# vanilladucky/sde_sampler_lrds

Hardware: NVIDIA B200
Metric: particle_steps_per_sec (higher is better)
Workload: dtype f32

## Files before the change

### sde_sampler_lrds_b200/csrc/lrds_rollout_mix.cuh

```cuda
#pragma once
#include "lrds_rollout_tc.cuh"

namespace lrds {

constexpr int MIX_MAX_WARPS = 16;
constexpr int MIX_TAIL_BYTES = 32;
constexpr float MIX_LOGIT_KAPPA = 9.5367431640625e-07f;
constexpr float MIX_LOGIT_KAPPA_C = 2.384185791015625e-07f;
constexpr float MIX_LOGIT_TAU = 2e-5f;

template <bool EUBO_, int TGT_, int REF_, bool EM_, bool DIS_ = false>
struct MixCfg {
  static constexpr bool kEubo = EUBO_, kEm = EM_, kDis = DIS_;
  static constexpr int kTgt = TGT_, kRef = REF_;
};
using MixBench = MixCfg<false, 1, 2, false>;

__host__ __device__ inline int mix_tc_config(const lrds_spec& s) {
  if (s.precision != LRDS_PRECISION_F16X3 || s.mlp.d_pad > 128 || gmm_full_on_path(s)) return -1;
  const bool tmix = s.ctrl_kind == LRDS_CTRL_SCORE && s.target.kind == LRDS_DISTR_GMM && s.target.gmm.M > 1 &&
                    s.target.gmm.M <= MIX_MAX_M && s.target.gmm.mix_tc != nullptr;
  const bool tdis = s.ctrl_kind >= LRDS_CTRL_CANCEL_DRIFT && s.target.kind == LRDS_DISTR_GMM && s.target.gmm.M > 1 &&
                    s.target.gmm.M <= MIX_MAX_M && s.target.gmm.mix_tc != nullptr;
  const bool tphi = s.ctrl_kind == LRDS_CTRL_SCORE && s.target.kind == LRDS_DISTR_PHI4;
  const bool tnone = s.ctrl_kind == LRDS_CTRL_CLIPPED &&
                     (s.target.kind != LRDS_DISTR_GMM || s.target.gmm.M <= MIX_MAX_M) && s.target.kind != LRDS_DISTR_LOGREG;
  const bool rnone = !s.has_ref_ctrl;
  const bool rmix = s.has_ref_ctrl && s.ref_t.M > 1 && s.ref_t.M <= MIX_MAX_M && s.ref_t.mix_tc != nullptr;
  const bool rgauss = s.has_ref_ctrl && s.ref_t.M == 1;
  const bool axpy = s.update_form == LRDS_UPDATE_AXPY && (s.ito_form == LRDS_ITO_SCALED || (rnone && s.ito_form != LRDS_ITO_EM));
  const bool em = s.update_form == LRDS_UPDATE_EM && (s.ito_form == LRDS_ITO_EM || (rnone && s.ito_form == LRDS_ITO_NONE));
  if (s.ref_0.M > MIX_MAX_M) return -1;
  if (s.target.kind == LRDS_DISTR_GMM && s.target.gmm.M > 1 && s.target.gmm.mix_tc == nullptr) return -1;
  if (s.kind == LRDS_ROLLOUT_EUBO_LINEAR) return (tmix && rmix && axpy) ? 1 : -1;
  if (s.kind != LRDS_ROLLOUT_LINEAR) return -1;
  if (tmix && rmix && axpy) return 0;
  if (tmix && rgauss && axpy) return 2;
  if (tmix && rgauss && em) return 3;
  if (tphi && rmix && axpy) return 4;
  if (tnone && rmix && axpy) return 5;
  if (tmix && rmix && em) return 6;
  if (tmix && rnone && em) return 7;
  if (tmix && rnone && axpy) return 8;
  if (tphi && rgauss && axpy) return 9;
  if (tdis && rnone && em) return 10;
  return -1;
}
__host__ __device__ inline bool mix_tc_applicable(const lrds_spec& s) { return mix_tc_config(s) >= 0; }

__device__ __forceinline__ float gmm_logp_any(const GmmView& g, int d, int dp, const Col4& x) {
  if (g.M == 1) {
    const int nq = (d + 3) >> 2;
    float q = 0.f;
    for (int c = 0; c < nq; ++c) quad4(q, x.ld4(c), g.mu.ld4(c), g.ivar.ld4(c));
    return g.glogc.ld1(0) - 0.5f * q;
  }
  float r[MIX_MAX_M];
  return gmm_pass1_pair(g, d, dp, x, r);
}

#ifdef LRDS_MIX_TIMING
static __device__ unsigned long long g_mix_timing[2 * 16 * 16];
struct MixTm {
  unsigned long long* w = nullptr;
  long long t;
  __device__ __forceinline__ void start() { t = clock64(); }
  __device__ __forceinline__ void mark(int i) {
    const long long n = clock64();
    if (w != nullptr && (threadIdx.x & 31) == 0) w[i] += (unsigned long long)(n - t);
    t = n;
  }
  __device__ __forceinline__ void count(int i, bool hit) {
    if (w != nullptr && (threadIdx.x & 31) == 0 && hit) w[i] += 1ull;
  }
};
#else
struct MixTm {
  __device__ __forceinline__ void start() {}
  __device__ __forceinline__ void mark(int) {}
  __device__ __forceinline__ void count(int, bool) {}
};
#endif

template <int PREC>
struct MixTc : TcMlp<PREC> {
  using Base = TcMlp<PREC>;
  static constexpr uint32_t kRCol = 0, kDCol = 32;
  uint32_t lbo, part_bytes;
  uint32_t lg_part;
  MixTm tm;

  __device__ __forceinline__ void logit(int which, uint32_t img, int col = -1) const {
    const uint32_t dcol = this->tm_tile + (col < 0 ? this->d_col() : (uint32_t)col) + (uint32_t)which * MIX_MAX_M;
    mma_passes<true, true>(dcol, this->tm_tile + this->a_col(0), this->tm_tile + this->a_col(1), 8u, img, lg_part,
                           2u * MIX_MAX_M * 16u, MIX_MAX_M * 16u, 128u, this->L.Kin / 16, ptx::make_idesc_f16(128, MIX_MAX_M));
  }
  template <bool TGT, bool REF>
  __device__ __forceinline__ void chunk(int c, uint32_t tgt_img, uint32_t ref_img, uint32_t col = kDCol, uint32_t rcol = kRCol) const {
    const uint32_t idesc = ptx::make_idesc_f16(128, 16);
#pragma unroll
    for (int which = TGT ? 0 : 1; which < (REF ? 2 : 1); ++which) {
      const uint32_t img = (which ? ref_img : tgt_img) + (uint32_t)c * 256u;
      const uint32_t dcol = this->tm_tile + col + which * 16;
      const uint32_t a_hi = this->tm_tile + rcol + which * 16, a_lo = a_hi + 8;
      const uint64_t b_hi = ptx::make_smem_desc(img, lbo, 128u), b_lo = ptx::make_smem_desc(img + part_bytes, lbo, 128u);
      ptx::mma_bf16_ts(dcol, a_lo, b_hi, idesc, 0);
      ptx::mma_bf16_ts(dcol, a_hi, b_lo, idesc, 1);
      ptx::mma_bf16_ts(dcol, a_hi, b_hi, idesc, 1);
    }
  }

  static __device__ __forceinline__ void pack_r(const float (&r)[MIX_MAX_M], uint32_t (&p)[16]) {
#pragma unroll
    for (int i = 0; i < 8; ++i) {
      u64 hi, lo;
      f2::split(f2::pack(r[2 * i], r[2 * i + 1]), hi, lo);
      float h0, h1, l0, l1;
      f2::unpack(hi, h0, h1);
      f2::unpack(lo, l0, l1);
      p[i] = ptx::pack_f16x2(h0, h1);
      p[8 + i] = ptx::pack_f16x2(l0, l1);
    }
  }
  __device__ __forceinline__ void store_r(int which, const uint32_t (&p)[16], uint32_t rcol = kRCol) {
    ptx::tmem_st16(this->tm_lane + rcol + which * 16, p);
  }
  __device__ __forceinline__ void load_chunk(uint32_t (&m)[32]) {
    ptx::tmem_ld32(this->tm_lane + kDCol, m);
    ptx::tmem_wait_ld();
  }

  static __device__ __forceinline__ bool softmax_logits(const uint32_t* acc, const PPtr<true>& tail, float xnorm, uint32_t (&p)[16]) {
    float r[MIX_MAX_M];
    const float4 t2 = tail.ld4(MIX_MAX_M / 4);
#pragma unroll
    for (int q = 0; q < MIX_MAX_M / 4; ++q) {
      const float4 c = tail.ld4(q);
      r[4 * q + 0] = fmaf(__uint_as_float(acc[4 * q + 0]), t2.x, c.x);
      r[4 * q + 1] = fmaf(__uint_as_float(acc[4 * q + 1]), t2.x, c.y);
      r[4 * q + 2] = fmaf(__uint_as_float(acc[4 * q + 2]), t2.x, c.z);
      r[4 * q + 3] = fmaf(__uint_as_float(acc[4 * q + 3]), t2.x, c.w);
    }
    float mx = r[0];
#pragma unroll
    for (int i = 1; i < MIX_MAX_M; ++i) mx = fmaxf(mx, r[i]);
    float s = 0.f;
#pragma unroll
    for (int mb = 0; mb < MIX_MAX_M / 4; ++mb) {
#pragma unroll
      for (int i = 0; i < 4; ++i) r[4 * mb + i] = __expf(r[4 * mb + i] - mx);
      s += (r[4 * mb] + r[4 * mb + 1]) + (r[4 * mb + 2] + r[4 * mb + 3]);
    }
    const float inv = 1.0f / s;
#pragma unroll
    for (int i = 0; i < MIX_MAX_M; ++i) r[i] *= inv;
    pack_r(r, p);
    const float eps = fmaf(MIX_LOGIT_KAPPA * xnorm, t2.y, MIX_LOGIT_KAPPA_C * t2.z);
    const float amb = fminf(1.0f, 4.0f * (s - 1.0f) * inv);
    return eps * amb <= MIX_LOGIT_TAU && xnorm < 3.0e4f;
  }

  template <bool BIAS_SH, class S0, class S1>
  __device__ __forceinline__ void hidden_ws(const float* __restrict__ bias1, S0&& slot0, S1&& slot1) {
    const TcLayout& L = this->L;
    this->issue(L.off_in, L.Kin, C);
    tm.mark(1);
    slot0();
    tm.mark(2);
    const float* bh = reinterpret_cast<const float*>(this->img + L.off_bhid);
    const int nh = L.nh;
    for (int l = 0; l <= nh; ++l) {
      if (l == 1) {
        slot1();
        tm.mark(5);
      }
      this->wait();
      tm.mark(l == 0 ? 3 : l == 1 ? 6 : 8);
      if (l == 0) this->template epilogue_f16<!BIAS_SH>(bias1, 0);
      else this->template epilogue_f16<false>(bh + (l - 1) * C, l);
      if (l < nh) this->issue(L.off_hid + (uint32_t)(l * C * C * L.es), C, C);
      else this->issue(L.off_out, C, L.Nout);
      tm.mark(l == 0 ? 4 : 7);
    }
    if (nh == 0) slot1();
    this->wait();
    tm.mark(8);
  }
};

template <bool RMIX>
__device__ __forceinline__ void mix_load_step(const lrds_spec& s, const StageLayout& SL, uint8_t* stage, int k) {
  uint64_t* sbar = reinterpret_cast<uint64_t*>(stage) + (k & 1);
  uint8_t* dst = stage + SL.off_buf + (k & 1) * SL.buf_bytes;
  const bool tgt = k == 0 && SL.tgt_bytes;
  ptx::mbar_expect_tx(sbar, SL.buf_bytes + (tgt ? SL.tgt_bytes : 0u));
  if (tgt) {
    stage_gmm(stage + SL.off_tgt, gmm_at(s.target.gmm, 0), SL.tgt_logc_bytes, SL.tgt_param_bytes, sbar);
    ptx::bulk_g2s(stage + SL.off_tgt + SL.tgt_logc_bytes + SL.tgt_param_bytes, static_cast<const uint8_t*>(s.target.gmm.mix_tc),
                  SL.tgt_mix_bytes, sbar);
  }
  stage_step(dst, s, SL, k, sbar);
  if constexpr (RMIX)
    ptx::bulk_g2s(dst + SL.row_bytes + SL.ref_logc_bytes + SL.ref_param_bytes,
                  static_cast<const uint8_t*>(s.ref_t.mix_tc) + (int64_t)k * s.ref_t.step_stride_mix_tc, SL.ref_mix_bytes, sbar);
}

template <int PREC, class CFG>
__device__ __forceinline__ void rollout_body_mix(const RolloutArgs& a, float* smem, uint8_t* stage, uint32_t* step_cnt, const int nwarps,
                                                 MixTc<PREC>& mlp) {
  constexpr bool EUBO = CFG::kEubo, TMIX = CFG::kTgt == 1, TPHI = CFG::kTgt == 2, RMIX = CFG::kRef == 2, RGAUSS = CFG::kRef == 1, EM = CFG::kEm, DIS = CFG::kDis;
  const lrds_spec& s = a.s;
  const int NT = nwarps * 32;
  const int tid = threadIdx.x;
  const int b_raw = blockIdx.x * NT + tid;
  const bool live = b_raw < s.B;
  const int b = live ? b_raw : s.B - 1;
  const int d = s.d, dp = s.mlp.d_pad, K = s.K;
  const ColLayout L = col_layout(s, true);
  const Particle P = make_particle(smem, L, NT, tid);

  for (int j = 0; j < dp; ++j) P.x(j) = (j < d) ? __ldg(a.x0 + (int64_t)b * d + j) : 0.f;
  if (!EUBO && a.traj_out != nullptr && live)
    for (int j = 0; j < d; ++j) a.traj_out[(int64_t)b * d + j] = P.x(j);

  CtrlConst cc = ctrl_const(s);
  const GmmView tv0 = gmm_at(s.target.gmm, 0);
  const StageLayout SL = stage_layout(s, 2, true);
  uint64_t* sbar = reinterpret_cast<uint64_t*>(stage);
  const uint32_t mix_off_t = SL.tgt_logc_bytes + SL.tgt_param_bytes;
  const uint32_t mix_off_r = SL.row_bytes + SL.ref_logc_bytes + SL.ref_param_bytes;
  const int Mt = TMIX ? s.target.gmm.M : s.ref_t.M;
  const uint32_t contr_bytes = gmm_mix_contr_bytes(Mt, dp), lg_part = gmm_mix_logit_part_bytes(Mt, dp);
  const uint32_t lg_tail_off = contr_bytes + 2u * lg_part;
  const GmmViewT<true> tv = staged_view(stage + SL.off_tgt, tv0, SL.tgt_logc_bytes, SL.tgt_param_bytes);
  const uint32_t tgt_img = ptx::smem_u32(stage + SL.off_tgt + mix_off_t);
  mlp.lbo = (uint32_t)(2 * dp) * 16u;
  mlp.part_bytes = (contr_bytes - 16u) / 2u;
  mlp.lg_part = lg_part;
  auto target_logp = [&]() -> float {
    if (s.target.kind == LRDS_DISTR_GMM) {
      if (s.target.gmm.M == 1) return gmm_logp_any(tv0, d, dp, P.x);
      float rt[MIX_MAX_M];
      return gmm_pass1_pair(tv, d, dp, P.x, rt);
    }
    if (s.target.kind == LRDS_DISTR_PHI4) return phi4_logp(s.target.phi4, d, P.x);
    return 0.f;
  };
  const float coef = s.target.phi4.a * (float)d, beta = s.target.phi4.beta;
  const u64 p0 = f2::pk(-beta * s.target.phi4.b / coef), p1 = f2::pk(beta / coef), p3 = f2::pk(-beta / coef),
            pn = f2::pk(beta * coef), m2 = f2::pk(-2.0f);
  const int nchunk = dp / JC;
  const int nq = (d + 3) >> 2;
  float rnd = 0.f;
  __syncwarp();
  if constexpr (EUBO) {
    ptx::mbar_wait(sbar, 0);
    const float lref = gmm_logp_any(gmm_at(s.ref_0, 0), d, dp, P.x);
    rnd = lref - clipf(target_logp(), s.clip_target);
  }

  mlp.tm.start();
  for (int k = 0; k < K; ++k) {
    ptx::mbar_wait(sbar + (k & 1), (uint32_t)(k >> 1) & 1u);
    mlp.tm.mark(0);
    const uint8_t* buf = stage + SL.off_buf + (k & 1) * SL.buf_bytes;
    const float* row = reinterpret_cast<const float*>(buf);
    const PPtr<true> rowp{ptx::smem_u32(buf)};
    const GmmViewT<true> rv = staged_view(buf + SL.row_bytes, gmm_at(s.ref_t, k), SL.ref_logc_bytes, SL.ref_param_bytes);
    const uint32_t ref_img = ptx::smem_u32(buf + mix_off_r);
    const float A = rowp.ld1(LRDS_STEP_A), Bc = rowp.ld1(LRDS_STEP_B), Cc = rowp.ld1(LRDS_STEP_C);
    const float wcost = rowp.ld1(LRDS_STEP_W_COST), wito = rowp.ld1(LRDS_STEP_W_ITO);
    const float gamma = rowp.ld1(LRDS_STEP_GAMMA);
    const float ust = TMIX ? *reinterpret_cast<const float*>(stage + SL.off_tgt + mix_off_t + contr_bytes - 16u) : 1.0f;
    const float usr = RMIX ? *reinterpret_cast<const float*>(buf + mix_off_r + contr_bytes - 16u) : 1.0f;
    const GmmView rg = gmm_at(s.ref_t, k);

    if constexpr (EUBO) {
      const u64 mean2 = f2::pk(rowp.ld1(LRDS_STEP_EU_A)), std2 = f2::pk(rowp.ld1(LRDS_STEP_EU_B));
      for (int c = 0; c < nchunk; ++c) {
        float z[JC];
        noise_chunk(a, k, b, c * JC, z);
        const ulonglong2 xa = P.x.ldu(2 * c), xb = P.x.ldu(2 * c + 1);
        P.x.stu(2 * c, ulonglong2{f2::fma(std2, f2::pack(z[0], z[1]), f2::mul(xa.x, mean2)),
                                  f2::fma(std2, f2::pack(z[2], z[3]), f2::mul(xa.y, mean2))});
        P.x.stu(2 * c + 1, ulonglong2{f2::fma(std2, f2::pack(z[4], z[5]), f2::mul(xb.x, mean2)),
                                      f2::fma(std2, f2::pack(z[6], z[7]), f2::mul(xb.y, mean2))});
      }
    }
    mlp.store_x(P.x);
    uint32_t rt_p[16], rr_p[16];
    bool need_t = TMIX, need_r = RMIX;
    bool ok_t = false, ok_r = false;
    if constexpr (TMIX || RMIX) {
      const PPtr<true> tail_t{tgt_img + lg_tail_off}, tail_r{ref_img + lg_tail_off};
      const bool lg_t = TMIX && tail_t.ld1(MIX_MAX_M + 3) != 0.f, lg_r = RMIX && tail_r.ld1(MIX_MAX_M + 3) != 0.f;
      if (lg_t || lg_r) {
        mlp.arrive_issue([&]() {
          if (lg_t) mlp.logit(0, tgt_img + contr_bytes);
          if (lg_r) mlp.logit(1, ref_img + contr_bytes);
        });
        u64 n2 = 0;
        for (int c = 0; c < nq; ++c) {
          const ulonglong2 xv = P.x.ldu(c);
          n2 = f2::fma(xv.x, xv.x, n2);
          n2 = f2::fma(xv.y, xv.y, n2);
        }
        const float xnorm = sqrtf(f2::hsum1(n2));
        mlp.wait();
        uint32_t lg[32];
        ptx::tmem_ld32(mlp.tm_lane + mlp.d_col(), lg);
        ptx::tmem_wait_ld();
        if (lg_t) {
          ok_t = mlp.softmax_logits(lg, tail_t, xnorm, rt_p);
          need_t = __any_sync(0xffffffffu, !ok_t);
        }
        if (lg_r) {
          ok_r = mlp.softmax_logits(lg + MIX_MAX_M, tail_r, xnorm, rr_p);
          need_r = __any_sync(0xffffffffu, !ok_r);
        }
      }
    }
    mlp.tm.count(14, need_t);
    mlp.tm.count(15, need_r);
    mlp.template hidden_ws<true>(
        row + LRDS_STEP_BIAS1,
        [&]() {
          if constexpr (TMIX) {
            if (need_t) {
              float r[MIX_MAX_M];
              uint32_t p[16];
              gmm_pass1_pair(tv, d, dp, P.x, r);
              mlp.pack_r(r, p);
#pragma unroll
              for (int i = 0; i < 16; ++i) rt_p[i] = ok_t ? rt_p[i] : p[i];
            }
          }
        },
        [&]() {
          if constexpr (RMIX) {
            if (need_r) {
              float r[MIX_MAX_M];
              uint32_t p[16];
              gmm_pass1_pair(rv, d, dp, P.x, r);
              mlp.pack_r(r, p);
#pragma unroll
              for (int i = 0; i < 16; ++i) rr_p[i] = ok_r ? rr_p[i] : p[i];
            }
          }
        });
    if constexpr (TMIX) mlp.store_r(0, rt_p);
    if constexpr (RMIX) mlp.store_r(1, rr_p);
    mlp.arrive_issue([&]() { mlp.template chunk<TMIX, RMIX>(0, tgt_img, ref_img); });
    mlp.tm.mark(9);
    const float dt = EM ? rowp.ld1(LRDS_STEP_DT) : 0.f, sqdt = EM ? rowp.ld1(LRDS_STEP_SQRT_DT) : 0.f;
    const u64 A2 = f2::pk(EM ? 1.0f - A * dt : A), B2 = f2::pk(EM ? Bc * dt : Bc), C2 = f2::pk(EM ? Bc * sqdt : Cc);
    const u64 usr2 = f2::pk(usr), R2 = f2::pk((EM ? Cc * dt : Bc) * usr);
    const bool lerp = DIS && s.ctrl_kind == LRDS_CTRL_LERP;
    const float gsc = DIS ? rowp.ld1(LRDS_STEP_GSCALE) : 1.0f, wl = DIS ? rowp.ld1(LRDS_STEP_LERP) : 0.f;
    const u64 cx2 = f2::pk(DIS ? rowp.ld1(LRDS_STEP_CX) : 0.f), ust2 = f2::pk(ust);
    const u64 wl2 = f2::pk(wl < 0.5f ? wl : -(1.0f - wl));
    const GmmView pg = gmm_at(s.ref_0, 0);
    const u64 gs2 = f2::pk(((cc.scale_score * gamma) * gsc) * (lerp ? 1.0f : ust));
    const float bts = lerp ? cc.bound_score : cc.bound_score / ust;
    const float wz = EM ? (s.ito_form == LRDS_ITO_NONE ? 0.f : sqdt)
                     : (RMIX || RGAUSS || s.ito_form == LRDS_ITO_SCALED) ? wito
                     : s.ito_form == LRDS_ITO_DDS ? rowp.ld1(LRDS_STEP_SIGU) * wito
                                                  : 0.f;
    u64 su2 = 0, sito = 0;
    float xm = 0.f;
    for (int c = 0; c < nchunk; ++c) {
      const int j0 = c * JC;
      uint32_t m[32];
      mlp.wait();
      mlp.tm.mark(10);
      mlp.load_chunk(m);
      if (c + 1 < nchunk) mlp.arrive_issue([&]() { mlp.template chunk<TMIX, RMIX>(c + 1, tgt_img, ref_img); });
      mlp.tm.mark(11);
      const ulonglong2 xa = P.x.ldu(2 * c), xb = P.x.ldu(2 * c + 1);
      const u64 X[4] = {xa.x, xa.y, xb.x, xb.y};
      u64 U[4], XN[4];
      float z[JC];
      mlp.out_chunk2(j0, U);
      noise_chunk(a, k, b, j0, z);
      float xs[JC + 2];
      if constexpr (TPHI) {
        xs[0] = xm;
#pragma unroll
        for (int q = 0; q < 4; ++q) f2::unpack(X[q], xs[1 + 2 * q], xs[2 + 2 * q]);
        xs[JC + 1] = (j0 + JC < dp) ? P.x(j0 + JC) : 0.f;
        xm = xs[JC];
      }
      u64 GM[4], GI[4];
      if constexpr (RGAUSS) {
        const ulonglong2 g0 = rg.mu.ld2(2 * c), g1 = rg.mu.ld2(2 * c + 1), i0 = rg.ivar.ld2(2 * c), i1 = rg.ivar.ld2(2 * c + 1);
        GM[0] = g0.x; GM[1] = g0.y; GM[2] = g1.x; GM[3] = g1.y;
        GI[0] = i0.x; GI[1] = i0.y; GI[2] = i1.x; GI[3] = i1.y;
      }
      if constexpr (DIS) {
        if (lerp) {
          const ulonglong2 g0 = pg.mu.ld2(2 * c), g1 = pg.mu.ld2(2 * c + 1), i0 = pg.ivar.ld2(2 * c), i1 = pg.ivar.ld2(2 * c + 1);
          GM[0] = g0.x; GM[1] = g0.y; GM[2] = g1.x; GM[3] = g1.y;
          GI[0] = i0.x; GI[1] = i0.y; GI[2] = i1.x; GI[3] = i1.y;
        }
      }
#pragma unroll
      for (int q = 0; q < 4; ++q) {
        const u64 ta = f2::pack(__uint_as_float(m[2 * q]), __uint_as_float(m[2 * q + 1]));
        const u64 tb = f2::pack(__uint_as_float(m[8 + 2 * q]), __uint_as_float(m[9 + 2 * q]));
        const u64 ra = f2::pack(__uint_as_float(m[16 + 2 * q]), __uint_as_float(m[17 + 2 * q]));
        const u64 rb = f2::pack(__uint_as_float(m[24 + 2 * q]), __uint_as_float(m[25 + 2 * q]));
        float t0 = 0.f, t1 = 0.f, u0, u1;
        if constexpr (TMIX) f2::unpack(f2::fma(X[q], ta, tb), t0, t1);
        if constexpr (DIS) {
          if (lerp) {
            const u64 tt = f2::mul(f2::pack(t0, t1), ust2);
            const u64 pr = f2::mul(f2::fma(X[q], f2::pk(-1.0f), GM[q]), GI[q]);
            const u64 df = f2::fma(pr, f2::pk(-1.0f), tt);
            f2::unpack(f2::fma(df, wl2, wl < 0.5f ? pr : tt), t0, t1);
          }
        }
        if constexpr (TPHI) {
          const u64 nb = f2::pack(xs[2 * q] + xs[2 * q + 2], xs[2 * q + 1] + xs[2 * q + 3]);
          const u64 t = f2::fma(X[q], f2::fma(f2::mul(X[q], X[q]), p3, p1), f2::fma(pn, f2::fma(X[q], m2, nb), p0));
          f2::unpack(t, t0, t1);
          if (j0 + JC > d) {
            if (j0 + 2 * q >= d) t0 = 0.f;
            if (j0 + 2 * q + 1 >= d) t1 = 0.f;
          }
        }
        f2::unpack(U[q], u0, u1);
        const u64 uc = f2::pack(clipb(u0, cc.bound_model), clipb(u1, cc.bound_model));
        u64 v = uc;
        if constexpr (DIS) v = f2::fma(X[q], cx2, v);
        if constexpr (TMIX || TPHI) v = f2::fma(f2::pack(clipb(t0, bts), clipb(t1, bts)), gs2, v);
        const u64 rraw = RMIX ? f2::fma(X[q], ra, rb) : RGAUSS ? f2::mul(f2::fma(X[q], f2::pk(-1.0f), GM[q]), GI[q]) : 0ull;
        const u64 z2 = f2::pack(z[2 * q], z[2 * q + 1]);
        if constexpr (EUBO) {
          su2 = f2::fma(v, f2::fma(v, f2::pk(0.5f), f2::mul(rraw, usr2)), su2);
          sito = f2::fma(v, z2, sito);
          continue;
        }
        su2 = f2::fma(v, v, su2);
        sito = f2::fma(v, z2, sito);
        if constexpr (!RMIX && !RGAUSS) {
          XN[q] = f2::fma(C2, z2, f2::fma(A2, X[q], f2::mul(B2, v)));
        } else if constexpr (EM) {
          XN[q] = f2::fma(C2, z2, f2::fma(A2, X[q], f2::fma(R2, rraw, f2::mul(B2, v))));
        } else {
          const u64 rv2 = f2::fma(rraw, usr2, v);
          XN[q] = f2::fma(C2, z2, f2::fma(A2, X[q], f2::mul(B2, rv2)));
        }
      }
      if constexpr (EUBO) {
        mlp.tm.mark(12);
        continue;
      }
      P.x.stu(2 * c, ulonglong2{XN[0], XN[1]});
      P.x.stu(2 * c + 1, ulonglong2{XN[2], XN[3]});
      if (a.traj_out != nullptr && live) {
        float xn[JC];
#pragma unroll
        for (int q = 0; q < 4; ++q) f2::unpack(XN[q], xn[2 * q], xn[2 * q + 1]);
        store_traj(a, k + 1, b, j0, xn);
      }
      mlp.tm.mark(12);
    }
    if constexpr (EUBO) {
      rnd -= f2::hsum1(su2) * wcost;
      rnd -= f2::hsum1(sito) * wito;
    } else {
      rnd += wcost * f2::hsum1(su2);
      rnd += wz * f2::hsum1(sito);
    }
    __syncwarp();
    if ((tid & 31) == 0) {
      const uint32_t old = ptx::atom_add_acq_rel(step_cnt + (k & 1), 1u);
      if (old == (uint32_t)((k >> 1) * nwarps + nwarps - 1) && k + 2 < K) mix_load_step<RMIX>(s, SL, stage, k + 2);
    }
    mlp.tm.mark(13);
  }
  __syncwarp();
  if constexpr (!EUBO) {
    const float lref = s.init_cost ? a.rnd_out[b] : gmm_logp_any(gmm_at(s.ref_0, 0), d, dp, P.x);
    rnd += lref - clipf(target_logp(), s.clip_target);
  }

  float xsum = 0.f;
  if (live) {
    a.rnd_out[b] = rnd;
    if (a.x_out != nullptr)
      for (int j = 0; j < d; ++j) {
        const float v = P.x(j);
        xsum += v;
        a.x_out[(int64_t)b * d + j] = v;
      }
  }
  report_status(s, live, mlp.saturated(), !isfinite(rnd + xsum));
}

template <int PREC, class CFG>
__device__ __forceinline__ void mix_aux_issuer(const RolloutArgs& a, uint8_t* stage, MixTc<PREC>& mlp) {
  constexpr bool TMIX = CFG::kTgt == 1, RMIX = CFG::kRef == 2;
  const lrds_spec& s = a.s;
  const int dp = s.mlp.d_pad, K = s.K, nchunk = dp / JC, nh = mlp.L.nh;
  const StageLayout SL = stage_layout(s, 2, true);
  uint64_t* sbar = reinterpret_cast<uint64_t*>(stage);
  const uint32_t mix_off_t = SL.tgt_logc_bytes + SL.tgt_param_bytes;
  const uint32_t mix_off_r = SL.row_bytes + SL.ref_logc_bytes + SL.ref_param_bytes;
  const int Mt = TMIX ? s.target.gmm.M : s.ref_t.M;
  const uint32_t contr_bytes = gmm_mix_contr_bytes(Mt, dp), lg_part = gmm_mix_logit_part_bytes(Mt, dp);
  const uint32_t lg_tail_off = contr_bytes + 2u * lg_part;
  const uint32_t tgt_img = ptx::smem_u32(stage + SL.off_tgt + mix_off_t);
  mlp.lbo = (uint32_t)(2 * dp) * 16u;
  mlp.part_bytes = (contr_bytes - 16u) / 2u;
  mlp.lg_part = lg_part;
  const TcLayout& L = mlp.L;
  for (int k = 0; k < K; ++k) {
    ptx::mbar_wait(sbar + (k & 1), (uint32_t)(k >> 1) & 1u);
    const uint8_t* buf = stage + SL.off_buf + (k & 1) * SL.buf_bytes;
    const uint32_t ref_img = ptx::smem_u32(buf + mix_off_r);
    if constexpr (TMIX || RMIX) {
      const PPtr<true> tail_t{tgt_img + lg_tail_off}, tail_r{ref_img + lg_tail_off};
      const bool lg_t = TMIX && tail_t.ld1(MIX_MAX_M + 3) != 0.f, lg_r = RMIX && tail_r.ld1(MIX_MAX_M + 3) != 0.f;
      if (lg_t || lg_r)
        mlp.issue_when_ready([&]() {
          if (lg_t) mlp.logit(0, tgt_img + contr_bytes);
          if (lg_r) mlp.logit(1, ref_img + contr_bytes);
        });
    }
    mlp.issue_when_ready([&]() { mlp.gemm(L.off_in, L.Kin, C); });
    for (int l = 0; l < nh; ++l) mlp.issue_when_ready([&]() { mlp.gemm(L.off_hid + (uint32_t)(l * C * C * L.es), C, C); });
    mlp.issue_when_ready([&]() { mlp.gemm(L.off_out, C, L.Nout); });
    for (int c = 0; c < nchunk; ++c) mlp.issue_when_ready([&]() { mlp.template chunk<TMIX, RMIX>(c, tgt_img, ref_img); });
  }
}

template <int PREC, class CFG>
__global__ void __launch_bounds__(MIX_MAX_WARPS * 32, 1)
rollout_mix_kernel(const RolloutArgs a, const uint8_t* __restrict__ image, const uint32_t tmem_cols, const int nwarps) {
  extern __shared__ __align__(128) uint8_t smem_raw[];
  constexpr bool RMIX = CFG::kRef == 2;
  const lrds_spec& s = a.s;
  const TcLayout TL = tc_layout(s.d, s.mlp.num_hidden, PREC);
  const int tid = threadIdx.x;
  const int warp = __shfl_sync(0xffffffffu, tid >> 5, 0);
  const bool has_aux = (int)(blockDim.x >> 5) > nwarps;
  uint64_t* bars = reinterpret_cast<uint64_t*>(smem_raw + TL.bytes);
  uint32_t* cnts = reinterpret_cast<uint32_t*>(smem_raw + TL.bytes + TC_TAIL_BYTES);
  uint8_t* stage = smem_raw + TL.bytes + TC_TAIL_BYTES + MIX_TAIL_BYTES;
  const StageLayout SL = stage_layout(s, 2, true);
  float* cols = reinterpret_cast<float*>(stage + ((SL.total + 15u) & ~15u));
  auto steps01 = [&]() {
    for (int k = 0; k < 2 && k < s.K; ++k) mix_load_step<RMIX>(s, SL, stage, k);
  };
  const uint32_t tmem = __shfl_sync(
      0xffffffffu, tc_cta_begin(smem_raw, TL, image, tmem_cols, warp, 5, reinterpret_cast<uint64_t*>(stage), 2, cnts, 6, 0u, steps01), 0);
  const bool aux = warp == nwarps;
  const int tile = aux ? (nwarps - 1) >> 2 : warp >> 2;
  const int tile_warps = min(4, nwarps - 4 * tile);
  uint32_t issue_mask = ((warp & 3) == tile_warps - 1 ? 1u : 0u) | ((warp & 3) == max(tile_warps - 2, 0) ? 2u : 0u);
  if (has_aux && tile_warps < 4) issue_mask = 0u;
  MixTc<PREC> mlp;
  mlp.init(TL, smem_raw, tmem + (uint32_t)(tile * TL.tile_cols), warp, bars + 1 + tile, cnts + tile, (uint32_t)tile_warps, issue_mask,
           s.mlp.d_pad);
#ifdef LRDS_MIX_TIMING
  unsigned long long* tmw = reinterpret_cast<unsigned long long*>(cols + (size_t)col_layout(s, true).total * 32 * nwarps) + warp * 16;
  if ((tid & 31) < 16) tmw[tid & 31] = 0;
  __syncwarp();
  mlp.tm.w = tmw;
#endif
  if (aux) mix_aux_issuer<PREC, CFG>(a, stage, mlp);
  else rollout_body_mix<PREC, CFG>(a, cols, stage, cnts + 4, nwarps, mlp);
#ifdef LRDS_MIX_TIMING
  __syncwarp();
  if ((blockIdx.x == 0 || blockIdx.x == gridDim.x / 2) && (tid & 31) < 16)
    g_mix_timing[((blockIdx.x ? 1 : 0) * 16 + warp) * 16 + (tid & 31)] = tmw[tid & 31];
#endif
  tc_cta_end(warp, tmem, tmem_cols);
}

inline bool plan_rollout_mix(const lrds_spec& s, int smem_cap, int sms, TcPlan* out) {
  if (!mix_tc_applicable(s)) return false;
  const TcLayout TL = tc_layout(s.d, s.mlp.num_hidden, s.precision);
  if (TL.tile_cols > 512 || TL.parts * TL.a_cols < 64) return false;
  const ColLayout CL = col_layout(s, true);
  size_t fixed = (size_t)TL.bytes + TC_TAIL_BYTES + MIX_TAIL_BYTES + ((stage_layout(s, 2, true).total + 15u) & ~15u);
#ifdef LRDS_MIX_TIMING
  fixed += 16 * 16 * 8;
#endif
  const size_t per_warp = (size_t)CL.total * 32 * sizeof(float);
  if (fixed + per_warp > (size_t)smem_cap) return false;
  int wmax = (int)(((size_t)smem_cap - fixed) / per_warp);
  wmax = wmax < MIX_MAX_WARPS ? wmax : MIX_MAX_WARPS;
  wmax = wmax < 4 * (512 / TL.tile_cols) ? wmax : 4 * (512 / TL.tile_cols);
  const int need = (s.B + 31) / 32;
  const int w = plan_warps(need, sms, wmax);
  out->warps = w;
  out->grid = (need + w - 1) / w;
  out->staged = 2;
  out->tmem_cols = plan_tmem_cols((w + 3) / 4 * TL.tile_cols);
  out->smem = fixed + per_warp * w;
  return true;
}

template <class CFG>
int launch_mix_cfg(const RolloutArgs& a, const TcPlan& p, cudaStream_t st) {
  const int aux = (p.warps % 4 != 0 && p.warps < MIX_MAX_WARPS) ? 1 : 0;
  return launch_tc(rollout_mix_kernel<LRDS_PRECISION_F16X3, CFG>, "mixture tensor-core rollout", a, p, (p.warps + aux) * 32, st,
                   p.tmem_cols, p.warps);
}

}
```

### sde_sampler_lrds_b200/csrc/lrds_rollout_simt.cuh

```cuda
#pragma once
#include "lrds_device.cuh"
#include "lrds_tc_ptx.cuh"

namespace lrds {

struct RolloutArgs {
  lrds_spec s;
  const float* x0;
  const float* noise;
  uint64_t seed;
  uint64_t particle_offset;
  float* x_out;
  float* rnd_out;
  float* traj_out;
};

__device__ __forceinline__ void report_status(const lrds_spec& s, bool live, bool saturated, bool nonfinite) {
  if (s.status != nullptr && live) {
    if (saturated) atomicAdd(s.status, 1u);
    if (nonfinite) atomicAdd(s.status + 1, 1u);
  }
}

struct ColLayout {
  int x, act, rt, rr, rh, g, us, tsd, db, total;
};

__host__ __device__ inline bool ref_t_full(const lrds_spec& s) { return s.has_ref_ctrl && s.ref_t.layout == LRDS_GMM_FULL; }
__host__ __device__ inline bool gmm_full_on_path(const lrds_spec& s) {
  return ref_t_full(s) || s.ref_0.layout == LRDS_GMM_FULL || (s.target.kind == LRDS_DISTR_GMM && s.target.gmm.layout == LRDS_GMM_FULL);
}

__host__ __device__ inline ColLayout col_layout(const lrds_spec& s, bool mix_tc = false) {
  ColLayout L{};
  int off = 0;
  const int dp = s.mlp.d_pad;
  L.x = off; off += dp;
  L.act = off;
  if (s.precision == LRDS_PRECISION_FP32_SIMT) off += C;
  L.rt = off;
  const bool tfull = s.target.kind == LRDS_DISTR_GMM && s.target.gmm.layout == LRDS_GMM_FULL;
  if (!mix_tc && !tfull && s.target.kind == LRDS_DISTR_GMM && s.target.gmm.M > 1) off += (s.target.gmm.M + 3) / 4 * 4;
  L.rr = off;
  L.rh = off;
  if (ref_t_full(s) || tfull) {
    L.rh = off + dp;
    off += 2 * dp;
    if (s.ref_0.layout != LRDS_GMM_FULL && s.ref_0.M > 1 && s.ref_0.M > 2 * dp) off += (s.ref_0.M + 3) / 4 * 4 - 2 * dp;
  } else if (!mix_tc) {
    int m = 0;
    if (s.has_ref_ctrl && s.ref_t.M > 1) m = s.ref_t.M;
    if (s.ref_0.layout != LRDS_GMM_FULL && s.ref_0.M > 1 && s.ref_0.M > m) m = s.ref_0.M;
    off += (m + 3) / 4 * 4;
  }
  L.g = off;
  if (s.target.kind == LRDS_DISTR_LOGREG) off += s.target.logreg.n_pad;
  L.us = off; L.tsd = off; L.db = off;
  if (s.kind == LRDS_ROLLOUT_CMCD || s.kind == LRDS_ROLLOUT_EUBO_CMCD) {
    L.us = off; off += dp;
    L.tsd = off; off += dp;
    L.db = off; off += dp;
  } else if (s.kind == LRDS_ROLLOUT_EUBO_LINEAR) {
    L.db = off; off += dp;
  }
  L.total = off;
  return L;
}

struct Particle {
  Col4 x, rt, rr, rh;
  Col g, us, tsd, db;
};

__device__ __forceinline__ Particle make_particle(float* smem, const ColLayout& L, int NT, int tid) {
  Particle P;
  P.x = Col4{smem + L.x * NT + 4 * tid, 4 * NT};
  P.rt = Col4{smem + L.rt * NT + 4 * tid, 4 * NT};
  P.rr = Col4{smem + L.rr * NT + 4 * tid, 4 * NT};
  P.rh = Col4{smem + L.rh * NT + 4 * tid, 4 * NT};
  P.g = Col{smem + L.g * NT + tid, NT};
  P.us = Col{smem + L.us * NT + tid, NT};
  P.tsd = Col{smem + L.tsd * NT + tid, NT};
  P.db = Col{smem + L.db * NT + tid, NT};
  return P;
}

struct StageLayout {
  uint32_t tgt_logc_bytes, tgt_param_bytes, tgt_bytes;
  uint32_t ref_logc_bytes, ref_param_bytes, row_bytes;
  uint32_t tgt_mix_bytes, ref_mix_bytes;
  uint32_t buf_bytes, off_tgt, off_buf, total;
};
__host__ __device__ inline uint32_t gmm_mix_contr_bytes(int M, int d_pad) {
  return 2u * (uint32_t)((M + 15) / 16 * 2) * (uint32_t)(2 * d_pad) * 16u + 16u;
}
__host__ __device__ inline uint32_t gmm_mix_logit_part_bytes(int M, int d_pad) {
  return (uint32_t)((M + 15) / 16 * 16) * (uint32_t)((d_pad + 15) / 16 * 16) * 2u;
}
__host__ __device__ inline uint32_t gmm_mix_tc_bytes(int M, int d_pad) {
  return gmm_mix_contr_bytes(M, d_pad) + 2u * gmm_mix_logit_part_bytes(M, d_pad) + (uint32_t)((M + 15) / 16 * 16) * 4u + 16u;
}

__host__ __device__ inline StageLayout stage_layout(const lrds_spec& s, int level, bool mix_tc = false) {
  StageLayout L{};
  const uint32_t dp = (uint32_t)s.mlp.d_pad;
  if (level >= 2 && s.target.kind == LRDS_DISTR_GMM && s.target.gmm.M > 1) {
    L.tgt_logc_bytes = (uint32_t)((s.target.gmm.M + 3) / 4 * 4) * 4u;
    L.tgt_param_bytes = (uint32_t)((s.target.gmm.M + 3) / 4) * dp * 32u;
    if (mix_tc) L.tgt_mix_bytes = gmm_mix_tc_bytes(s.target.gmm.M, s.mlp.d_pad);
    L.tgt_bytes = L.tgt_logc_bytes + L.tgt_param_bytes + L.tgt_mix_bytes;
  }
  if (s.has_ref_ctrl && s.ref_t.M > 1 && !ref_t_full(s)) {
    L.ref_logc_bytes = (uint32_t)((s.ref_t.M + 3) / 4 * 4) * 4u;
    L.ref_param_bytes = (uint32_t)((s.ref_t.M + 3) / 4) * dp * 32u;
    if (mix_tc) L.ref_mix_bytes = gmm_mix_tc_bytes(s.ref_t.M, s.mlp.d_pad);
  }
  L.row_bytes = LRDS_STEP_STRIDE * 4u;
  L.buf_bytes = L.row_bytes + L.ref_logc_bytes + L.ref_param_bytes + L.ref_mix_bytes;
  L.off_tgt = 16;
  L.off_buf = L.off_tgt + L.tgt_bytes;
  L.total = L.off_buf + 2u * L.buf_bytes;
  return L;
}

__device__ __forceinline__ void stage_gmm(uint8_t* dst, const GmmView& g, uint32_t logc_bytes, uint32_t param_bytes,
                                          uint64_t* bar) {
  ptx::bulk_g2s(dst, g.logc.p, logc_bytes, bar);
  ptx::bulk_g2s(dst + logc_bytes, g.sn.p, param_bytes, bar);
}
__device__ __forceinline__ void stage_step(uint8_t* dst, const lrds_spec& s, const StageLayout& L, int k, uint64_t* bar) {
  ptx::bulk_g2s(dst, s.steps + (int64_t)k * LRDS_STEP_STRIDE, L.row_bytes, bar);
  if (L.ref_param_bytes) stage_gmm(dst + L.row_bytes, gmm_at(s.ref_t, k), L.ref_logc_bytes, L.ref_param_bytes, bar);
}
__device__ __forceinline__ GmmViewT<true> staged_view(const uint8_t* src, const GmmView& g, uint32_t logc_bytes,
                                                     uint32_t param_bytes) {
  GmmViewT<true> v;
  const uint32_t a = ptx::smem_u32(src);
  v.M = g.M;
  v.logc = PPtr<true>{a};
  v.sn = PPtr<true>{a + logc_bytes};
  v.glogc = g.glogc;
  v.mu = g.mu;
  v.ivar = g.ivar;
  return v;
}

template <int UPDATE = -1, int ITO = -1, int TARGET = -1, int SCORE = -1, int REF = -1, int MIX = 0>
struct LinearTraits {
  static constexpr bool kMix = MIX != 0;
  static constexpr int kUpdate = UPDATE;
  static constexpr int kIto = ITO;
  static constexpr int kTarget = TARGET;
  static constexpr int kScore = SCORE;
  static constexpr int kRef = REF;
};
using RuntimeTraits = LinearTraits<>;
__host__ __device__ inline int ref_class(const lrds_spec& s) {
  return !s.has_ref_ctrl ? 0 : (ref_t_full(s) ? 3 : (s.ref_t.M > 1 ? 2 : 1));
}
template <class TR>
__host__ __device__ inline bool traits_match(const lrds_spec& s) {
  return (TR::kUpdate < 0 || TR::kUpdate == s.update_form) && (TR::kIto < 0 || TR::kIto == s.ito_form) &&
         (TR::kTarget < 0 || TR::kTarget == s.target.kind) &&
         (TR::kScore < 0 || (s.ctrl_kind <= LRDS_CTRL_SCORE && TR::kScore == (s.ctrl_kind == LRDS_CTRL_SCORE))) &&
         (TR::kRef < 0 || TR::kRef == ref_class(s)) && (TR::kRef < 0 || !gmm_full_on_path(s)) &&
         (!TR::kMix || ((s.target.kind != LRDS_DISTR_GMM || s.target.gmm.M > 1) && (!s.has_ref_ctrl || s.ref_t.M > 1)));
}

struct SimtMlp {
  static constexpr bool kPipe = true;
  const lrds_mlp& w;
  Col act;
  template <bool BIAS_SH>
  __device__ __forceinline__ void hidden(const float* __restrict__ bias1, const Col4& x) {
    mlp_hidden<BIAS_SH>(w, bias1, x, act);
  }
  __device__ __forceinline__ void out_chunk(int j0, float (&out)[JC]) { mlp_out_chunk(w, act, j0, out); }
  __device__ __forceinline__ bool saturated() const { return false; }
};

template <bool PIPE, bool MIX = false, bool SH>
__device__ __forceinline__ float target_pass1(const lrds_spec& s, int kind, const GmmViewT<SH>& tv, const Particle& P,
                                              bool want_logp) {
  const lrds_distr& t = s.target;
  if (kind == LRDS_DISTR_GMM) return gmm_pass1<PIPE, MIX>(tv, s.d, s.mlp.d_pad, P.x, P.rt);
  if (kind == LRDS_DISTR_LOGREG) return logreg_pass1(t.logreg, s.d, P.x, P.g, want_logp);
  if (kind == LRDS_DISTR_PHI4) return want_logp ? phi4_logp(t.phi4, s.d, P.x) : 0.f;
  return 0.f;
}

template <bool PIPE, bool MIX = false, bool SH>
__device__ __forceinline__ void target_score_chunk(const lrds_spec& s, int kind, const GmmViewT<SH>& tv, const Particle& P,
                                                   const float (&xr)[JC], float xm, float xp, int j0, float (&out)[JC]) {
  const lrds_distr& t = s.target;
  if (kind == LRDS_DISTR_GMM) {
    gmm_score_chunk<PIPE, MIX>(tv, s.d, s.mlp.d_pad, xr, P.rt, j0, out);
  } else if (kind == LRDS_DISTR_LOGREG) {
    logreg_score_chunk(t.logreg, s.d, s.mlp.d_pad, xr, P.g, j0, out);
  } else if (kind == LRDS_DISTR_PHI4) {
    const float coef = t.phi4.a * (float)s.d;
#pragma unroll
    for (int c = 0; c < JC; ++c) {
      const float left = (c == 0) ? xm : xr[c - 1];
      const float right = (c == JC - 1) ? xp : xr[c + 1];
      const int j = j0 + c;
      out[c] = (j < s.d) ? phi4_score_1(t.phi4, coef, left, xr[c], (j == s.d - 1) ? 0.f : right) : 0.f;
    }
  } else {
#pragma unroll
    for (int c = 0; c < JC; ++c) out[c] = 0.f;
  }
}

__device__ __forceinline__ void load_chunk(const Col& v, int j0, float (&out)[JC]) {
#pragma unroll
  for (int c = 0; c < JC; ++c) out[c] = v(j0 + c);
}
__device__ __forceinline__ void load_chunk(const Col4& v, int j0, float (&out)[JC]) {
  const float4 a = v.ld4(j0 >> 2), b = v.ld4((j0 >> 2) + 1);
  out[0] = a.x; out[1] = a.y; out[2] = a.z; out[3] = a.w; out[4] = b.x; out[5] = b.y; out[6] = b.z; out[7] = b.w;
}
__device__ __forceinline__ void store_chunk(const Col4& v, int j0, const float (&in)[JC]) {
  v.st4(j0 >> 2, make_float4(in[0], in[1], in[2], in[3]));
  v.st4((j0 >> 2) + 1, make_float4(in[4], in[5], in[6], in[7]));
}

template <bool PIPE, bool SH, class F>
__device__ __forceinline__ void target_score_loop(const lrds_spec& s, int kind, const GmmViewT<SH>& tv, const Particle& P,
                                                  F&& consume) {
  const int dp = s.mlp.d_pad;
  float xm = 0.f;
  for (int j0 = 0; j0 < dp; j0 += JC) {
    float xr[JC], ts[JC];
    load_chunk(P.x, j0, xr);
    const float xp = (j0 + JC < dp) ? P.x(j0 + JC) : 0.f;
    target_score_chunk<PIPE>(s, kind, tv, P, xr, xm, xp, j0, ts);
    xm = xr[JC - 1];
    consume(j0, xr, ts);
  }
}

struct ParticleThread {
  int b;
  bool live;
  Particle P;
};
__device__ __forceinline__ ParticleThread particle_thread(const lrds_spec& s, float* smem) {
  const int NT = blockDim.x, tid = threadIdx.x;
  const int b_raw = blockIdx.x * NT + tid;
  const bool live = b_raw < s.B;
  return ParticleThread{live ? b_raw : s.B - 1, live, make_particle(smem, col_layout(s), NT, tid)};
}

constexpr int MIX_MAX_M = 16;

template <bool SH>
__device__ __forceinline__ float gmm_pass1_pair(const GmmViewT<SH>& g, int d, int dp, const Col4& x, float (&r)[MIX_MAX_M]) {
  const int lane = threadIdx.x & 31, h = lane >> 4;
  const int nq = (d + 3) >> 2;
  const int rowq = dp >> 2;
  const int M4 = (g.M + 3) >> 2;
  const int nb = (M4 + 1) >> 1;
  const int b0 = h * nb;
  const Col4 xo{x.p + ((lane ^ 16) - lane) * 4, x.stride};
  const int blk0 = min(b0, M4 - 1), blk1 = min(b0 + 1, M4 - 1);
  PPtr<SH> p0 = g.sn + blk0 * rowq * 32, p1 = g.sn + blk1 * rowq * 32;
  u64 qa[8] = {0, 0, 0, 0, 0, 0, 0, 0}, qb[8] = {0, 0, 0, 0, 0, 0, 0, 0};
  auto block = [&](const PPtr<SH>& p, const ulonglong2& xa, const ulonglong2& xb, int o) {
#pragma unroll
    for (int i = 0; i < 4; ++i) {
      const ulonglong2 sv = p.ld2(2 * i), nv = p.ld2(2 * i + 1);
      const u64 a0 = f2::fma(xa.x, sv.x, nv.x), a1 = f2::fma(xa.y, sv.y, nv.y);
      const u64 c0 = f2::fma(xb.x, sv.x, nv.x), c1 = f2::fma(xb.y, sv.y, nv.y);
      qa[o + i] = f2::fma(a0, a0, qa[o + i]);
      qb[o + i] = f2::fma(c0, c0, qb[o + i]);
      qa[o + i] = f2::fma(a1, a1, qa[o + i]);
      qb[o + i] = f2::fma(c1, c1, qb[o + i]);
    }
  };
  if (nb > 1) {
    for (int c = 0; c < nq; ++c, p0 = p0 + 32, p1 = p1 + 32) {
      const ulonglong2 xa = x.ldu(c), xb = xo.ldu(c);
      block(p0, xa, xb, 0);
      block(p1, xa, xb, 4);
    }
  } else {
    for (int c = 0; c < nq; ++c, p0 = p0 + 32) {
      const ulonglong2 xa = x.ldu(c), xb = xo.ldu(c);
      block(p0, xa, xb, 0);
    }
  }
  float own[8], oth[8];
  {
    const float4 l0 = g.logc.ld4(blk0), l1 = g.logc.ld4(blk1);
    const float lc[8] = {l0.x, l0.y, l0.z, l0.w, l1.x, l1.y, l1.z, l1.w};
    const bool v0 = b0 < M4, v1 = nb > 1 && b0 + 1 < M4;
#pragma unroll
    for (int k = 0; k < 8; ++k) {
      const bool v = k < 4 ? v0 : v1;
      float ax, ay, bx, by;
      f2::unpack(qa[k], ax, ay);
      f2::unpack(qb[k], bx, by);
      own[k] = v ? lc[k] - 0.5f * (ax + ay) : -INFINITY;
      oth[k] = v ? lc[k] - 0.5f * (bx + by) : -INFINITY;
    }
  }
#pragma unroll
  for (int k = 0; k < 8; ++k) oth[k] = __shfl_xor_sync(0xffffffffu, oth[k], 16);
  if (nb > 1) {
#pragma unroll
    for (int k = 0; k < 8; ++k) {
      r[k] = h ? oth[k] : own[k];
      r[8 + k] = h ? own[k] : oth[k];
    }
  } else {
#pragma unroll
    for (int k = 0; k < 4; ++k) {
      r[k] = h ? oth[k] : own[k];
      r[4 + k] = h ? own[k] : oth[k];
    }
#pragma unroll
    for (int k = 8; k < MIX_MAX_M; ++k) r[k] = -INFINITY;
  }
  float mx = r[0];
#pragma unroll
  for (int i = 1; i < MIX_MAX_M; ++i) mx = fmaxf(mx, r[i]);
  float s = 0.f;
#pragma unroll
  for (int mb = 0; mb < MIX_MAX_M / 4; ++mb) {
#pragma unroll
    for (int i = 0; i < 4; ++i) r[4 * mb + i] = __expf(r[4 * mb + i] - mx);
    s += (r[4 * mb] + r[4 * mb + 1]) + (r[4 * mb + 2] + r[4 * mb + 3]);
  }
  const float inv = 1.0f / s;
#pragma unroll
  for (int i = 0; i < MIX_MAX_M; ++i) r[i] *= inv;
  return mx + __logf(s);
}

struct CtrlConst {
  float bound_model, bound_score, scale_score;
  bool score;
  int d;
  int kind;
};
__device__ __forceinline__ CtrlConst ctrl_const(const lrds_spec& s) {
  return CtrlConst{clip_bound(s.clip_model), clip_bound(s.clip_score), s.scale_score, s.ctrl_kind != LRDS_CTRL_CLIPPED, s.d,
                   s.ctrl_kind};
}
template <class MLP>
__device__ __forceinline__ void ctrl_chunk(const CtrlConst& cc, MLP& mlp, int j0, const float (&ts)[JC], float gamma,
                                           float (&u)[JC]) {
  mlp.out_chunk(j0, u);
#pragma unroll
  for (int c = 0; c < JC; ++c) {
    float v = clipb(u[c], cc.bound_model);
    if (cc.score) v = v + (cc.scale_score * clipb(ts[c], cc.bound_score)) * gamma;
    u[c] = (j0 + c < cc.d) ? v : 0.f;
  }
}

struct CtrlStep {
  float gamma, cx, gscale, w;
};
__device__ __forceinline__ CtrlStep ctrl_step(const float* __restrict__ row) {
  return CtrlStep{__ldg(row + LRDS_STEP_GAMMA), __ldg(row + LRDS_STEP_CX), __ldg(row + LRDS_STEP_GSCALE), __ldg(row + LRDS_STEP_LERP)};
}
__device__ __forceinline__ float lerpf(float a, float b, float w) {
  return w < 0.5f ? a + w * (b - a) : b - (b - a) * (1.0f - w);
}
template <class MLP>
__device__ __forceinline__ void ctrl_chunk_dis(const CtrlConst& cc, MLP& mlp, int j0, const float (&ts)[JC],
                                               const float (&xr)[JC], const float (&ps)[JC], const CtrlStep& st, float (&u)[JC]) {
  mlp.out_chunk(j0, u);
#pragma unroll
  for (int c = 0; c < JC; ++c) {
    float v = clipb(u[c], cc.bound_model);
    const float sc = cc.kind == LRDS_CTRL_LERP ? lerpf(ps[c], ts[c], st.w) : ts[c];
    const float t = (cc.scale_score * clipb(sc, cc.bound_score)) * st.gamma;
    if (cc.kind == LRDS_CTRL_CANCEL_DRIFT) v = v + st.cx * xr[c];
    v = v + st.gscale * t;
    u[c] = (j0 + c < cc.d) ? v : 0.f;
  }
}

__device__ __forceinline__ void noise_chunk(const RolloutArgs& a, int step, int b, int j0, float (&z)[JC]) {
  if (a.noise != nullptr) {
    const float* p = a.noise + ((int64_t)step * a.s.B + b) * a.s.d + j0;
#pragma unroll
    for (int c = 0; c < JC; ++c) z[c] = (j0 + c < a.s.d) ? __ldg(p + c) : 0.f;
  } else {
    float z4[4];
    const uint32_t pidx = (uint32_t)(a.particle_offset + (uint64_t)b);
    normals4(a.seed, pidx, (uint32_t)step, (uint32_t)(j0 >> 2), 0u, z4);
    z[0] = z4[0]; z[1] = z4[1]; z[2] = z4[2]; z[3] = z4[3];
    normals4(a.seed, pidx, (uint32_t)step, (uint32_t)(j0 >> 2) + 1u, 0u, z4);
    z[4] = z4[0]; z[5] = z4[1]; z[6] = z4[2]; z[7] = z4[3];
    if (j0 + JC > a.s.d) {
#pragma unroll
      for (int c = 0; c < JC; ++c)
        if (j0 + c >= a.s.d) z[c] = 0.f;
    }
  }
}

__device__ __forceinline__ void store_traj(const RolloutArgs& a, int row, int b, int j0, const float (&v)[JC]) {
  float* p = a.traj_out + ((int64_t)row * a.s.B + b) * a.s.d + j0;
#pragma unroll
  for (int c = 0; c < JC; ++c)
    if (j0 + c < a.s.d) p[c] = v[c];
}

__device__ __forceinline__ float langevin_drift(const lrds_spec& s, float ts, float ps, float frac) {
  float dr = ts * frac + ps * (1.0f - frac);
  dr *= 0.5f * s.cmcd_diff * s.cmcd_diff;
  return clipf(dr, s.cmcd_clip);
}

template <bool PIPE>
__device__ __forceinline__ float ref0_log_prob(const lrds_spec& s, const Particle& P) {
  if (s.ref_0.layout == LRDS_GMM_FULL) return gmm_full_pass<false>(gmm_full_at(s.ref_0, 0), s.d, s.mlp.d_pad, P.x, P.rr, P.rh);
  return gmm_pass1<PIPE>(gmm_at(s.ref_0, 0), s.d, s.mlp.d_pad, P.x, P.rr);
}

template <int KIND, int STAGE, class TR = RuntimeTraits, class MLP>
__device__ __forceinline__ void rollout_body(const RolloutArgs& a, float* smem, uint8_t* stage, MLP& mlp) {
  constexpr bool PIPE = MLP::kPipe;
  const lrds_spec& s = a.s;
  const int NT = blockDim.x;
  const int tid = threadIdx.x;
  const int b_raw = blockIdx.x * NT + tid;
  const bool live = b_raw < s.B;
  const int b = live ? b_raw : s.B - 1;
  const int d = s.d, dp = s.mlp.d_pad, K = s.K;
  const ColLayout L = col_layout(s);
  const Particle P = make_particle(smem, L, NT, tid);

  for (int j = 0; j < dp; ++j) P.x(j) = (j < d) ? __ldg(a.x0 + (int64_t)b * d + j) : 0.f;
  if (a.traj_out != nullptr && live)
    for (int j = 0; j < d; ++j) a.traj_out[(int64_t)b * d + j] = P.x(j);

  const int tkind = TR::kTarget >= 0 ? TR::kTarget : s.target.kind;
  const bool score_ctrl = TR::kScore >= 0 ? TR::kScore != 0 : s.ctrl_kind != LRDS_CTRL_CLIPPED;
  const bool dis_ctrl = TR::kScore < 0 && s.ctrl_kind >= LRDS_CTRL_CANCEL_DRIFT;
  const bool has_ref = TR::kRef >= 0 ? TR::kRef != 0 : s.has_ref_ctrl != 0;
  const int update_form = TR::kUpdate >= 0 ? TR::kUpdate : s.update_form;
  const int ito_form = TR::kIto >= 0 ? TR::kIto : s.ito_form;
  const bool need_nbr = tkind == LRDS_DISTR_PHI4;
  const bool rfull = TR::kRef < 0 && has_ref && s.ref_t.layout == LRDS_GMM_FULL;
  CtrlConst cc = ctrl_const(s);
  cc.score = score_ctrl;
  const GmmView tv0 = gmm_at(s.target.gmm, 0);
  float rnd = 0.f;

  if constexpr (KIND == LRDS_ROLLOUT_LINEAR) {
    constexpr bool STAGED = STAGE > 0;
    constexpr bool SH = STAGED, TSH = STAGE > 1;
    const StageLayout SL = stage_layout(s, STAGE);
    uint64_t* sbar = reinterpret_cast<uint64_t*>(stage);
    GmmViewT<TSH> tv{};
    if constexpr (!TSH) tv = tv0;
    if constexpr (STAGED) {
      if (tid == 0) {
        ptx::mbar_init(sbar, 1);
        ptx::mbar_init(sbar + 1, 1);
        ptx::fence_mbar_init();
      }
      __syncthreads();
      if (tid == 0) {
        ptx::mbar_expect_tx(sbar, SL.tgt_bytes + SL.buf_bytes);
        if (SL.tgt_bytes) stage_gmm(stage + SL.off_tgt, tv0, SL.tgt_logc_bytes, SL.tgt_param_bytes, sbar);
        stage_step(stage + SL.off_buf, s, SL, 0, sbar);
      }
      if constexpr (TSH) tv = staged_view(stage + SL.off_tgt, tv0, SL.tgt_logc_bytes, SL.tgt_param_bytes);
    }
    for (int k = 0; k < K; ++k) {
      const float* row = s.steps + (int64_t)k * LRDS_STEP_STRIDE;
      GmmViewT<SH> rv{};
      PPtr<SH> rowp{};
      if constexpr (STAGED) {
        __syncthreads();
        if (tid == 0 && k + 1 < K) {
          ptx::mbar_expect_tx(sbar + ((k + 1) & 1), SL.buf_bytes);
          stage_step(stage + SL.off_buf + ((k + 1) & 1) * SL.buf_bytes, s, SL, k + 1, sbar + ((k + 1) & 1));
        }
        ptx::mbar_wait(sbar + (k & 1), (uint32_t)(k >> 1) & 1u);
        const uint8_t* buf = stage + SL.off_buf + (k & 1) * SL.buf_bytes;
        row = reinterpret_cast<const float*>(buf);
        rowp = PPtr<true>{ptx::smem_u32(buf)};
        if (has_ref && !rfull) rv = staged_view(buf + SL.row_bytes, gmm_at(s.ref_t, k), SL.ref_logc_bytes, SL.ref_param_bytes);
      } else {
        rowp = PPtr<false>{row};
        if (has_ref && !rfull) rv = gmm_at(s.ref_t, k);
      }
      const float A = rowp.ld1(LRDS_STEP_A), Bc = rowp.ld1(LRDS_STEP_B), Cc = rowp.ld1(LRDS_STEP_C);
      const float dt = rowp.ld1(LRDS_STEP_DT), sqdt = rowp.ld1(LRDS_STEP_SQRT_DT);
      const float wcost = rowp.ld1(LRDS_STEP_W_COST), wito = rowp.ld1(LRDS_STEP_W_ITO);
      const float gamma = rowp.ld1(LRDS_STEP_GAMMA), sigu = rowp.ld1(LRDS_STEP_SIGU);
      if (score_ctrl) target_pass1<PIPE, TR::kMix>(s, tkind, tv, P, false);
      if (rfull) gmm_full_pass<true>(gmm_full_at(s.ref_t, k), d, dp, P.x, P.rr, P.rh);
      else if (has_ref && (TR::kRef == 2 || rv.M > 1)) gmm_pass1<PIPE, TR::kMix>(rv, d, dp, P.x, P.rr);
      mlp.template hidden<SH>(row + LRDS_STEP_BIAS1, P.x);
      float su2 = 0.f, sito = 0.f, xm = 0.f;
      for (int j0 = 0; j0 < dp; j0 += JC) {
        float xr[JC], ts[JC], u[JC], rs[JC], z[JC], xn[JC];
        load_chunk(P.x, j0, xr);
        const float xp = (need_nbr && j0 + JC < dp) ? P.x(j0 + JC) : 0.f;
        if (score_ctrl) target_score_chunk<PIPE, TR::kMix>(s, tkind, tv, P, xr, xm, xp, j0, ts);
        if (dis_ctrl) {
          float ps[JC] = {};
          if (cc.kind == LRDS_CTRL_LERP) gmm_score_chunk<false, false>(gmm_at(s.ref_0, 0), d, dp, xr, P.rr, j0, ps);
          ctrl_chunk_dis(cc, mlp, j0, ts, xr, ps, ctrl_step(s.steps + (int64_t)k * LRDS_STEP_STRIDE), u);
        } else {
          ctrl_chunk(cc, mlp, j0, ts, gamma, u);
        }
        if (rfull) load_chunk(P.rr, j0, rs);
        else if (has_ref) gmm_score_chunk<PIPE, TR::kMix>(rv, d, dp, xr, P.rr, j0, rs);
        noise_chunk(a, k, b, j0, z);
#pragma unroll
        for (int c = 0; c < JC; ++c) {
          const float r = has_ref ? rs[c] : 0.f;
          su2 = fmaf(u[c], u[c], su2);
          if (update_form == LRDS_UPDATE_AXPY) {
            xn[c] = (A * xr[c] + Bc * (r + u[c])) + Cc * z[c];
          } else {
            float drift = -(A * xr[c]);
            if (has_ref) drift += Cc * r;
            xn[c] = xr[c] + (drift + Bc * u[c]) * dt + Bc * (z[c] * sqdt);
          }
          if (ito_form == LRDS_ITO_SCALED) sito = fmaf(u[c], z[c], sito);
          else if (ito_form == LRDS_ITO_EM) sito = fmaf(u[c], z[c] * sqdt, sito);
          else if (ito_form == LRDS_ITO_DDS) sito += ((sigu * u[c]) * z[c]) * wito;
          if (j0 + c >= d) xn[c] = 0.f;
        }
        xm = xr[JC - 1];
        store_chunk(P.x, j0, xn);
        if (a.traj_out != nullptr && live) store_traj(a, k + 1, b, j0, xn);
      }
      rnd += wcost * su2;
      if (ito_form == LRDS_ITO_SCALED) rnd += wito * sito;
      else if (ito_form != LRDS_ITO_NONE) rnd += sito;
    }
    const float lref = s.init_cost ? a.rnd_out[b] : ref0_log_prob<PIPE>(s, P);
    const float ltgt = clipf(target_pass1<PIPE>(s, tkind, tv, P, true), s.clip_target);
    rnd += lref - ltgt;
  }

  if constexpr (KIND == LRDS_ROLLOUT_EUBO_LINEAR) {
    {
      const float lref = s.init_cost ? 0.f : ref0_log_prob<PIPE>(s, P);
      const float ltgt = clipf(target_pass1<PIPE>(s, tkind, tv0, P, true), s.clip_target);
      rnd = lref - ltgt;
    }
    for (int k = 0; k < K; ++k) {
      const float* row = s.steps + (int64_t)k * LRDS_STEP_STRIDE;
      const float mean = __ldg(row + LRDS_STEP_EU_A), stdf = __ldg(row + LRDS_STEP_EU_B);
      const float wx = __ldg(row + LRDS_STEP_EU_C), sig = __ldg(row + LRDS_STEP_B);
      const float wcost = __ldg(row + LRDS_STEP_W_COST), wito = __ldg(row + LRDS_STEP_W_ITO);
      const float gamma = __ldg(row + LRDS_STEP_GAMMA);
      for (int j0 = 0; j0 < dp; j0 += JC) {
        float z[JC];
        noise_chunk(a, k, b, j0, z);
#pragma unroll
        for (int c = 0; c < JC; ++c) {
          P.db(j0 + c) = z[c];
          P.x(j0 + c) = (j0 + c < d) ? fmaf(stdf, z[c], P.x(j0 + c) * mean) : 0.f;
        }
      }
      if (score_ctrl) target_pass1<PIPE>(s, tkind, tv0, P, false);
      GmmView rv{};
      if (rfull) {
        gmm_full_pass<true>(gmm_full_at(s.ref_t, k), d, dp, P.x, P.rr, P.rh);
      } else if (has_ref) {
        rv = gmm_at(s.ref_t, k);
        if (rv.M > 1) gmm_pass1<PIPE>(rv, d, dp, P.x, P.rr);
      }
      mlp.template hidden<false>(row + LRDS_STEP_BIAS1, P.x);
      float cost = 0.f, gx = 0.f, gz = 0.f, xm = 0.f;
      for (int j0 = 0; j0 < dp; j0 += JC) {
        float xr[JC], ts[JC], u[JC], rs[JC];
        load_chunk(P.x, j0, xr);
        const float xp = (need_nbr && j0 + JC < dp) ? P.x(j0 + JC) : 0.f;
        if (score_ctrl) target_score_chunk<PIPE>(s, tkind, tv0, P, xr, xm, xp, j0, ts);
        ctrl_chunk(cc, mlp, j0, ts, gamma, u);
        if (rfull) {
          load_chunk(P.rr, j0, rs);
        } else if (has_ref) {
          gmm_score_chunk<PIPE>(rv, d, dp, xr, P.rr, j0, rs);
        } else {
#pragma unroll
          for (int c = 0; c < JC; ++c) rs[c] = 0.f;
        }
#pragma unroll
        for (int c = 0; c < JC; ++c) {
          const float g = (s.update_form == LRDS_UPDATE_EM) ? u[c] / sig : u[c];
          cost = fmaf(g, rs[c] + 0.5f * g, cost);
          gx = fmaf(g, xr[c], gx);
          gz = fmaf(g, P.db(j0 + c), gz);
        }
        xm = xr[JC - 1];
      }
      rnd -= cost * wcost;
      if (s.update_form == LRDS_UPDATE_EM) rnd += gx * wx;
      rnd -= gz * wito;
    }
    if (s.init_cost) rnd += gmm_pass1<PIPE>(gmm_at(s.ref_0, 0), d, dp, P.x, P.rr);
  }

  if constexpr (KIND == LRDS_ROLLOUT_CMCD || KIND == LRDS_ROLLOUT_EUBO_CMCD) {
    constexpr bool EUBO = (KIND == LRDS_ROLLOUT_EUBO_CMCD);
    const GmmView prior = gmm_at(s.ref_0, 0);
    const float sg = s.cmcd_diff;
    auto eval_point = [&](int rowi, bool first, float dtk, float frac_for_drift, float& c2, float& cdb) {
      const float* row = s.steps + (int64_t)rowi * LRDS_STEP_STRIDE;
      const float gamma = __ldg(row + LRDS_STEP_GAMMA);
      target_pass1<PIPE>(s, tkind, tv0, P, false);
      mlp.template hidden<false>(row + LRDS_STEP_BIAS1, P.x);
      float xm = 0.f;
      for (int j0 = 0; j0 < dp; j0 += JC) {
        float xr[JC], ts[JC], u[JC];
        load_chunk(P.x, j0, xr);
        const float xp = (need_nbr && j0 + JC < dp) ? P.x(j0 + JC) : 0.f;
        target_score_chunk<PIPE>(s, tkind, tv0, P, xr, xm, xp, j0, ts);
        ctrl_chunk(cc, mlp, j0, ts, gamma, u);
#pragma unroll
        for (int c = 0; c < JC; ++c) {
          const int j = j0 + c;
          if (!first && j < d) {
            const float ps = -((xr[c] - prior.mu.ld1(j)) * prior.ivar.ld1(j));
            const float dnew = langevin_drift(s, ts[c], ps, frac_for_drift);
            const float cst = EUBO ? ((dnew + P.tsd(j)) / sg + u[c] - P.us(j))
                                   : ((P.tsd(j) + dnew) / sg + P.us(j) - u[c]);
            c2 = fmaf(cst, cst, c2);
            cdb = fmaf(cst, P.db(j), cdb);
          }
          P.us(j) = u[c];
          P.tsd(j) = (j < d) ? ts[c] : 0.f;
        }
        xm = xr[JC - 1];
      }
      (void)dtk;
    };
    float c2 = 0.f, cdb = 0.f;
    if constexpr (!EUBO) {
      rnd = gmm_pass1<PIPE>(prior, d, dp, P.x, P.rr);
      eval_point(0, true, 0.f, 0.f, c2, cdb);
      for (int k = 0; k < K; ++k) {
        const float* row = s.steps + (int64_t)k * LRDS_STEP_STRIDE;
        const float dt = __ldg(row + LRDS_STEP_DT), sqdt = __ldg(row + LRDS_STEP_SQRT_DT);
        const float fs = __ldg(row + LRDS_STEP_FRAC), ft = __ldg(row + LRDS_STEP_STRIDE + LRDS_STEP_FRAC);
        for (int j0 = 0; j0 < dp; j0 += JC) {
          float z[JC], xn[JC];
          noise_chunk(a, k, b, j0, z);
#pragma unroll
          for (int c = 0; c < JC; ++c) {
            const int j = j0 + c;
            float y = 0.f;
            if (j < d) {
              const float xj = P.x(j);
              const float ps = -((xj - prior.mu.ld1(j)) * prior.ivar.ld1(j));
              const float ds = langevin_drift(s, P.tsd(j), ps, fs);
              const float db = sqdt * z[c];
              y = xj + (ds + P.us(j) * sg) * dt + sg * db;
              P.tsd(j) = ds;
              P.db(j) = db;
            }
            xn[c] = y;
            P.x(j) = y;
          }
          if (a.traj_out != nullptr && live) store_traj(a, k + 1, b, j0, xn);
        }
        c2 = 0.f; cdb = 0.f;
        eval_point(k + 1, false, dt, ft, c2, cdb);
        rnd += 0.5f * c2 * dt;
        rnd += cdb;
      }
      rnd -= clipf(target_pass1<PIPE>(s, tkind, tv0, P, true), s.clip_target);
    } else {
      rnd = -clipf(target_pass1<PIPE>(s, tkind, tv0, P, true), s.clip_target);
      eval_point(K, true, 0.f, 0.f, c2, cdb);
      for (int i = 0; i < K; ++i) {
        const int kt = K - i, ks = K - 1 - i;
        const float* rows = s.steps + (int64_t)ks * LRDS_STEP_STRIDE;
        const float dt = __ldg(rows + LRDS_STEP_DT), sqdt = __ldg(rows + LRDS_STEP_SQRT_DT);
        const float ft = __ldg(s.steps + (int64_t)kt * LRDS_STEP_STRIDE + LRDS_STEP_FRAC);
        for (int j0 = 0; j0 < dp; j0 += JC) {
          float z[JC];
          noise_chunk(a, i, b, j0, z);
#pragma unroll
          for (int c = 0; c < JC; ++c) {
            const int j = j0 + c;
            float y = 0.f;
            if (j < d) {
              const float xj = P.x(j);
              const float ps = -((xj - prior.mu.ld1(j)) * prior.ivar.ld1(j));
              const float dtt = langevin_drift(s, P.tsd(j), ps, ft);
              const float db = sqdt * z[c];
              y = xj + (dtt - P.us(j) * sg) * dt + sg * db;
              P.tsd(j) = dtt;
              P.db(j) = db;
            }
            P.x(j) = y;
          }
        }
        c2 = 0.f; cdb = 0.f;
        eval_point(ks, false, dt, ft, c2, cdb);
        rnd -= 0.5f * c2 * dt;
        rnd -= cdb;
      }
      rnd += gmm_pass1<PIPE>(prior, d, dp, P.x, P.rr);
    }
  }

  float xsum = 0.f;
  if (live) {
    a.rnd_out[b] = rnd;
    if (a.x_out != nullptr)
      for (int j = 0; j < d; ++j) {
        const float v = P.x(j);
        xsum += v;
        a.x_out[(int64_t)b * d + j] = v;
      }
  }
  report_status(s, live, mlp.saturated(), !isfinite(rnd + xsum));
}

template <int KIND>
__global__ void __launch_bounds__(128) rollout_simt_kernel(const RolloutArgs a) {
  extern __shared__ float smem[];
  const ColLayout L = col_layout(a.s);
  SimtMlp mlp{a.s.mlp, Col{smem + L.act * blockDim.x + threadIdx.x, (int)blockDim.x}};
  rollout_body<KIND, 0, RuntimeTraits>(a, smem, nullptr, mlp);
}

}
```

### sde_sampler_lrds_b200/csrc/lrds_rollout_tc.cuh

```cuda
#pragma once
#include <cuda_fp16.h>

#include "lrds_internal.h"
#include "lrds_rollout_simt.cuh"
#include "lrds_tc_ptx.cuh"

namespace lrds {

constexpr int TC_MAX_WARPS = 16;
__host__ __device__ constexpr int tc_max_warps(int prec) {
  return prec == LRDS_PRECISION_TF32X3 ? 8 : prec == LRDS_PRECISION_F16X3 ? 12 : TC_MAX_WARPS;
}
constexpr int TC_TAIL_BYTES = 96;
constexpr float TC_ACT_SCALE = 64.f;
__host__ __device__ constexpr bool tc_is_x3(int prec) { return prec == LRDS_PRECISION_TF32X3 || prec == LRDS_PRECISION_F16X3; }
__host__ __device__ constexpr bool tc_is_half(int prec) { return prec == LRDS_PRECISION_BF16 || prec == LRDS_PRECISION_F16X3; }

struct TcLayout {
  int prec, parts, es, kstep;
  int Kin, Nout, nh;
  uint32_t part_bytes, off_in, off_hid, off_out;
  uint32_t off_bhid, off_bout, off_scale, bytes;
  int a_cols, d_cols, tile_cols;
};

__host__ __device__ inline TcLayout tc_layout(int d, int nh, int prec) {
  TcLayout L{};
  L.prec = prec;
  L.parts = tc_is_x3(prec) ? 2 : 1;
  L.es = tc_is_half(prec) ? 2 : 4;
  L.kstep = tc_is_half(prec) ? 16 : 8;
  L.Kin = (d + L.kstep - 1) / L.kstep * L.kstep;
  L.Nout = (d + 15) / 16 * 16;
  L.nh = nh;
  L.off_in = 0;
  L.off_hid = (uint32_t)(C * L.Kin * L.es);
  L.off_out = L.off_hid + (uint32_t)(nh * C * C * L.es);
  L.part_bytes = L.off_out + (uint32_t)(L.Nout * C * L.es);
  L.off_bhid = L.parts * L.part_bytes;
  L.off_bout = L.off_bhid + (uint32_t)((nh > 0 ? nh : 1) * C * 4);
  L.off_scale = L.off_bout + (uint32_t)(L.Nout * 4);
  L.bytes = L.off_scale + 64u;
  L.a_cols = (L.Kin > C ? L.Kin : C) * L.es / 4;
  L.d_cols = L.Nout > C ? L.Nout : C;
  L.tile_cols = L.parts * L.a_cols + L.d_cols;
  return L;
}

static __global__ void tc_scales_kernel(const lrds_mlp w, const TcLayout L, uint8_t* __restrict__ img) {
  __shared__ float red[32];
  float* sc = reinterpret_cast<float*>(img + L.off_scale);
  for (int l = 0; l < L.nh + 2; ++l) {
    const float* p = l == 0 ? w.w_in_t : (l <= L.nh ? w.w_hid_t + (int64_t)(l - 1) * C * C : w.w_out_t);
    const int n = l == 0 ? w.d * C : (l <= L.nh ? C * C : C * w.d_pad);
    float m = 0.f;
    for (int i = threadIdx.x; i < n; i += blockDim.x) m = fmaxf(m, fabsf(p[i]));
    m = block_reduce(m, MaxOp{}, 0.f, red);
    if (threadIdx.x == 0) {
      const int k = pow2_exponent_for(m);
      sc[l] = ldexpf(1.0f, k);
      sc[8 + l] = ldexpf(1.0f, -k) / (l == 0 ? 1.0f : TC_ACT_SCALE);
    }
  }
}

static __global__ void pack_tc_image_kernel(const lrds_mlp w, const TcLayout L, uint8_t* __restrict__ img) {
  const int E = 16 / L.es;
  const int n_in = C * L.Kin, n_hid = L.nh * C * C, n_out = L.Nout * C;
  const int total = n_in + n_hid + n_out;
  const float* sc = reinterpret_cast<const float*>(img + L.off_scale);
  for (int idx = blockIdx.x * blockDim.x + threadIdx.x; idx < total; idx += gridDim.x * blockDim.x) {
    float v;
    uint32_t off;
    int n, k, N, layer;
    if (idx < n_in) {
      n = idx / L.Kin; k = idx % L.Kin; N = C; off = L.off_in; layer = 0;
      v = k < w.d ? w.w_in_t[(int64_t)k * C + n] : 0.f;
    } else if (idx < n_in + n_hid) {
      const int r = idx - n_in, l = r / (C * C);
      n = (r / C) % C; k = r % C; N = C; off = L.off_hid + (uint32_t)(l * C * C * L.es); layer = 1 + l;
      v = w.w_hid_t[(int64_t)l * C * C + (int64_t)k * C + n];
    } else {
      const int r = idx - n_in - n_hid;
      n = r / C; k = r % C; N = L.Nout; off = L.off_out; layer = L.nh + 1;
      v = n < w.d_pad ? w.w_out_t[(int64_t)k * w.d_pad + n] : 0.f;
    }
    const uint32_t byte = off + (uint32_t)(k / E) * N * 16u + (uint32_t)n * 16u + (uint32_t)(k % E) * L.es;
    if (L.prec == LRDS_PRECISION_BF16) {
      *reinterpret_cast<uint16_t*>(img + byte) = (uint16_t)(ptx::pack_bf16x2(v, 0.f) & 0xFFFFu);
    } else if (L.prec == LRDS_PRECISION_F16X3) {
      put_hi_lo(img, L.part_bytes, byte, v * sc[layer]);
    } else {
      const float hi = ptx::to_tf32(v);
      *reinterpret_cast<float*>(img + byte) = hi;
      if (L.parts == 2) *reinterpret_cast<float*>(img + L.part_bytes + byte) = ptx::to_tf32(v - hi);
    }
  }
  float* bh = reinterpret_cast<float*>(img + L.off_bhid);
  float* bo = reinterpret_cast<float*>(img + L.off_bout);
  for (int i = blockIdx.x * blockDim.x + threadIdx.x; i < (L.nh > 0 ? L.nh : 1) * C; i += gridDim.x * blockDim.x)
    bh[i] = i < L.nh * C ? w.b_hid[i] : 0.f;
  for (int i = blockIdx.x * blockDim.x + threadIdx.x; i < L.Nout; i += gridDim.x * blockDim.x)
    bo[i] = i < w.d_pad ? w.b_out[i] : 0.f;
}

template <bool X3, bool UNROLL, bool TF32 = false>
__device__ __forceinline__ void mma_passes(uint32_t dcol, uint32_t a_hi, uint32_t a_lo, uint32_t a_step, uint32_t b, uint32_t b_part,
                                           uint32_t b_step, uint32_t lbo, uint32_t sbo, int ksteps, uint32_t idesc) {
  uint32_t acc = 0;
#pragma unroll(UNROLL ? 3 : 1)
  for (int pass = X3 ? 0 : 2; pass < 3; ++pass) {
    const uint32_t a = pass == 0 ? a_lo : a_hi;
    const uint32_t bb = b + (pass == 1 ? b_part : 0u);
    for (int ks = 0; ks < ksteps; ++ks) {
      const uint64_t bdesc = ptx::make_smem_desc(bb + (uint32_t)ks * b_step, lbo, sbo);
      if (TF32) ptx::mma_tf32_ts(dcol, a + (uint32_t)ks * a_step, bdesc, idesc, acc);
      else ptx::mma_bf16_ts(dcol, a + (uint32_t)ks * a_step, bdesc, idesc, acc);
      acc = 1;
    }
  }
}

template <class F>
__device__ __forceinline__ uint32_t tc_cta_begin(uint8_t* smem, const TcLayout& TL, const uint8_t* image, uint32_t tmem_cols,
                                                  int warp, int nbars, uint64_t* sbar, int nsbar, uint32_t* cnts, int ncnt,
                                                  uint32_t extra_bytes, F&& extra) {
  uint64_t* bars = reinterpret_cast<uint64_t*>(smem + TL.bytes);
  uint32_t* slot = reinterpret_cast<uint32_t*>(smem + TL.bytes + 48);
  if (warp == 0) ptx::tmem_alloc(slot, tmem_cols);
  if (threadIdx.x == 0) {
    for (int i = 0; i < nbars; ++i) ptx::mbar_init(bars + i, 1);
    for (int i = 0; i < nsbar; ++i) ptx::mbar_init(sbar + i, 1);
    for (int i = 0; i < ncnt; ++i) cnts[i] = 0u;
    ptx::fence_mbar_init();
  }
  ptx::tc_fence_before();
  __syncthreads();
  ptx::tc_fence_after();
  if (threadIdx.x == 0) {
    ptx::mbar_expect_tx(bars, TL.bytes + extra_bytes);
    ptx::bulk_g2s(smem, image, TL.bytes, bars);
    extra();
  }
  ptx::mbar_wait(bars, 0);
  return *slot;
}
__device__ __forceinline__ void tc_cta_end(int warp, uint32_t tmem, uint32_t tmem_cols) {
  ptx::tc_fence_before();
  __syncthreads();
  if (warp == 0) ptx::tmem_dealloc(tmem, tmem_cols);
}

template <int PREC>
struct TcMlp {
  static constexpr bool kX3 = tc_is_x3(PREC);
  static constexpr bool kHalf = tc_is_half(PREC);
  static constexpr bool kF16 = PREC == LRDS_PRECISION_F16X3;
  static constexpr bool kPipe = tc_max_warps(PREC) <= 8;
  TcLayout L;
  const uint8_t* img;
  uint32_t img_s;
  uint32_t tm_tile;
  uint32_t tm_lane;
  uint64_t* bar;
  uint32_t phase;
  uint32_t* cnt;
  uint32_t target;
  uint32_t tile_warps;
  uint32_t issue_mask;
  uint32_t hand;
  int dp;
  float vmax = 0.f, xmax = 0.f;
  __device__ __forceinline__ bool saturated() const { return kF16 && (vmax > F16X3_MAX_PREACT || xmax > F16X3_MAX_COORD); }

  __device__ __forceinline__ void init(const TcLayout& TL, const uint8_t* smem, uint32_t tmem_tile, int warp, uint64_t* tile_bar,
                                       uint32_t* tile_cnt, uint32_t warps, uint32_t mask, int d_pad) {
    L = TL;
    img = smem;
    img_s = ptx::smem_u32(smem);
    tm_tile = tmem_tile;
    tm_lane = tmem_tile + ((uint32_t)((warp & 3) * 32) << 16);
    bar = tile_bar;
    phase = 0;
    cnt = tile_cnt;
    target = 0u;
    tile_warps = warps;
    issue_mask = mask;
    hand = 0u;
    dp = d_pad;
  }

  static __device__ __forceinline__ uint32_t split_hi(float v) {
    if (kX3) return __float_as_uint(v) & 0xFFFFE000u;
    return __float_as_uint(ptx::to_tf32(v));
  }
  __device__ __forceinline__ uint32_t a_col(int part) const { return (uint32_t)(part * L.a_cols); }
  __device__ __forceinline__ uint32_t d_col() const { return (uint32_t)(L.parts * L.a_cols); }
  __device__ __forceinline__ float unscale(int layer) const {
    return reinterpret_cast<const float*>(img + L.off_scale)[8 + layer];
  }

  template <class F>
  __device__ __forceinline__ void arrive_issue(F&& f, uint64_t* done = nullptr) {
    ptx::tmem_wait_st();
    ptx::tc_fence_before();
    __syncwarp();
    if ((threadIdx.x & 31) == 0) ptx::red_add_release(cnt, 1u);
    const bool mine = (issue_mask >> (hand & 1u)) & 1u;
    ++hand;
    if (mine) issue_when_ready(f, done);
    else target += tile_warps;
  }
  template <class F>
  __device__ __forceinline__ void issue_when_ready(F&& f, uint64_t* done = nullptr) {
    target += tile_warps;
    while ((int32_t)(ptx::ld_acquire(cnt) - target) < 0) {
    }
    ptx::tc_fence_after();
    if (ptx::elect_one()) {
      f();
      ptx::mma_commit(done ? done : bar);
    }
    __syncwarp();
  }

  __device__ __forceinline__ void gemm(uint32_t b_off, int K, int N) const {
    const uint32_t idesc = PREC == LRDS_PRECISION_BF16 ? ptx::make_idesc_bf16(128, N)
                           : kF16                      ? ptx::make_idesc_f16(128, N)
                                                       : ptx::make_idesc_tf32(128, N);
    mma_passes<kX3, true, !kHalf>(tm_tile + d_col(), tm_tile + a_col(0), tm_tile + a_col(1), 8u, img_s + b_off, L.part_bytes,
                                  2u * (uint32_t)N * 16u, (uint32_t)N * 16u, 128u, K / L.kstep, idesc);
  }
  __device__ __forceinline__ void issue(uint32_t b_off, int K, int N) {
    arrive_issue([&]() { gemm(b_off, K, N); });
  }
  __device__ __forceinline__ void wait() {
    ptx::mbar_wait(bar, phase);
    phase ^= 1u;
    ptx::tc_fence_after();
  }

  __device__ __forceinline__ void store8(int c0, const float (&v)[8]) {
    uint32_t hi[8];
#pragma unroll
    for (int i = 0; i < 8; ++i) hi[i] = split_hi(v[i]);
    ptx::tmem_st8(tm_lane + a_col(0) + c0, hi);
    if (kX3) {
      uint32_t lo[8];
#pragma unroll
      for (int i = 0; i < 8; ++i) lo[i] = __float_as_uint(v[i] - __uint_as_float(hi[i]));
      ptx::tmem_st8(tm_lane + a_col(1) + c0, lo);
    }
  }
  __device__ __forceinline__ void store16_half(int c0, const float (&v)[16]) {
    uint32_t r[8];
    if (kF16) {
      uint32_t rl[8];
#pragma unroll
      for (int i = 0; i < 8; ++i) {
        u64 hi, lo;
        xmax = max3abs(xmax, v[2 * i], v[2 * i + 1]);
        f2::split(f2::pack(v[2 * i], v[2 * i + 1]), hi, lo);
        float h0, h1, l0, l1;
        f2::unpack(hi, h0, h1);
        f2::unpack(lo, l0, l1);
        r[i] = ptx::pack_f16x2(h0, h1);
        rl[i] = ptx::pack_f16x2(l0, l1);
      }
      ptx::tmem_st8(tm_lane + a_col(0) + c0, r);
      ptx::tmem_st8(tm_lane + a_col(1) + c0, rl);
    } else {
#pragma unroll
      for (int i = 0; i < 8; ++i) r[i] = ptx::pack_bf16x2(v[2 * i], v[2 * i + 1]);
      ptx::tmem_st8(tm_lane + a_col(0) + c0, r);
    }
  }

  __device__ __forceinline__ void store_x(const Col4& x, int g0 = 0, int gstep = 1) {
    if (kHalf) {
      for (int c0 = 8 * g0; c0 < L.Kin / 2; c0 += 8 * gstep) {
        float v[16];
#pragma unroll
        for (int h = 0; h < 2; ++h) {
          const int j0 = 2 * c0 + 8 * h;
          float4 a = make_float4(0.f, 0.f, 0.f, 0.f), b = a;
          if (j0 < dp) {
            a = x.ld4(j0 >> 2);
            b = x.ld4((j0 >> 2) + 1);
          }
          v[8 * h + 0] = a.x; v[8 * h + 1] = a.y; v[8 * h + 2] = a.z; v[8 * h + 3] = a.w;
          v[8 * h + 4] = b.x; v[8 * h + 5] = b.y; v[8 * h + 6] = b.z; v[8 * h + 7] = b.w;
        }
        store16_half(c0, v);
      }
    } else {
      for (int c0 = 8 * g0; c0 < L.Kin; c0 += 8 * gstep) {
        const float4 a = x.ld4(c0 >> 2), b = x.ld4((c0 >> 2) + 1);
        const float v[8] = {a.x, a.y, a.z, a.w, b.x, b.y, b.z, b.w};
        store8(c0, v);
      }
    }
  }

  template <bool GLOBAL_BIAS, int W = 32>
  __device__ __forceinline__ void epilogue_f16(const float* __restrict__ bias, int layer, int c_begin = 0, int c_end = C) {
    static_assert(W == 32 || W == 16, "tcgen05.ld / st widths");
    const u64 us2 = f2::pk(unscale(layer));
#pragma unroll 1
    for (int c0 = c_begin; c0 < c_end; c0 += W) {
      uint32_t r[W];
      if constexpr (W == 32) ptx::tmem_ld32(tm_lane + d_col() + c0, r);
      else ptx::tmem_ld16(tm_lane + d_col() + c0, r);
      ptx::tmem_wait_ld();
      const float4* b4 = reinterpret_cast<const float4*>(bias + c0);
      uint32_t ph[W / 2], pl[W / 2];
#pragma unroll
      for (int i = 0; i < W / 4; ++i) {
        const float4 b = GLOBAL_BIAS ? __ldg(b4 + i) : b4[i];
#pragma unroll
        for (int e = 0; e < 2; ++e) {
          const u64 acc = f2::pack(__uint_as_float(r[4 * i + 2 * e]), __uint_as_float(r[4 * i + 2 * e + 1]));
          const u64 v = f2::fma(acc, us2, e ? f2::pack(b.z, b.w) : f2::pack(b.x, b.y));
          {
            float va, vb;
            f2::unpack(v, va, vb);
            vmax = max3(vmax, va, vb);
          }
          const u64 g = gelu_pair(v, 5.0f, TC_ACT_SCALE);
          u64 hi, lo;
          f2::split(g, hi, lo);
          float h0, h1, l0, l1;
          f2::unpack(hi, h0, h1);
          f2::unpack(lo, l0, l1);
          ph[2 * i + e] = ptx::pack_f16x2(h0, h1);
          pl[2 * i + e] = ptx::pack_f16x2(l0, l1);
        }
      }
      if constexpr (W == 32) {
        ptx::tmem_st16(tm_lane + a_col(0) + c0 / 2, ph);
        ptx::tmem_st16(tm_lane + a_col(1) + c0 / 2, pl);
      } else {
        ptx::tmem_st8(tm_lane + a_col(0) + c0 / 2, ph);
        ptx::tmem_st8(tm_lane + a_col(1) + c0 / 2, pl);
      }
    }
  }

  template <bool GLOBAL_BIAS>
  __device__ __forceinline__ void epilogue(const float* __restrict__ bias, int layer) {
    if constexpr (kF16) {
      epilogue_f16<GLOBAL_BIAS>(bias, layer);
    } else {
#pragma unroll 1
      for (int c0 = 0; c0 < C; c0 += 32) {
        uint32_t r[32];
        ptx::tmem_ld32(tm_lane + d_col() + c0, r);
        ptx::tmem_wait_ld();
        float g[32];
        const float4* b4 = reinterpret_cast<const float4*>(bias + c0);
#pragma unroll
        for (int i = 0; i < 8; ++i) {
          const float4 b = GLOBAL_BIAS ? __ldg(b4 + i) : b4[i];
          gelu_exact2(__uint_as_float(r[4 * i + 0]) + b.x, __uint_as_float(r[4 * i + 1]) + b.y, g[4 * i + 0], g[4 * i + 1]);
          gelu_exact2(__uint_as_float(r[4 * i + 2]) + b.z, __uint_as_float(r[4 * i + 3]) + b.w, g[4 * i + 2], g[4 * i + 3]);
        }
        if (kHalf) {
          float lo16[16], hi16[16];
#pragma unroll
          for (int i = 0; i < 16; ++i) { lo16[i] = g[i]; hi16[i] = g[16 + i]; }
          store16_half(c0 / 2, lo16);
          store16_half(c0 / 2 + 8, hi16);
        } else {
          uint32_t hi[32];
#pragma unroll
          for (int i = 0; i < 32; ++i) hi[i] = split_hi(g[i]);
          ptx::tmem_st32(tm_lane + a_col(0) + c0, hi);
          if (kX3) {
#pragma unroll
            for (int i = 0; i < 32; ++i) hi[i] = __float_as_uint(g[i] - __uint_as_float(hi[i]));
            ptx::tmem_st32(tm_lane + a_col(1) + c0, hi);
          }
        }
      }
    }
  }

  template <bool BIAS_SH>
  __device__ __forceinline__ void hidden(const float* __restrict__ bias1, const Col4& x) {
    store_x(x);
    issue(L.off_in, L.Kin, C);
    const float* bh = reinterpret_cast<const float*>(img + L.off_bhid);
    for (int l = 0; l < L.nh; ++l) {
      wait();
      if (l == 0) epilogue<!BIAS_SH>(bias1, 0);
      else epilogue<false>(bh + (l - 1) * C, l);
      issue(L.off_hid + (uint32_t)(l * C * C * L.es), C, C);
    }
    wait();
    if (L.nh == 0) epilogue<!BIAS_SH>(bias1, 0);
    else epilogue<false>(bh + (L.nh - 1) * C, L.nh);
    issue(L.off_out, C, L.Nout);
    wait();
  }

  __device__ __forceinline__ void out_chunk2(int j0, u64 (&out)[JC / 2]) {
    uint32_t r[8];
    ptx::tmem_ld8(tm_lane + d_col() + j0, r);
    ptx::tmem_wait_ld();
    const ulonglong2* b2 = reinterpret_cast<const ulonglong2*>(img + L.off_bout + j0 * 4);
    const ulonglong2 a = b2[0], b = b2[1];
    const u64 us2 = f2::pk(unscale(L.nh + 1));
    out[0] = f2::fma(f2::pack(__uint_as_float(r[0]), __uint_as_float(r[1])), us2, a.x);
    out[1] = f2::fma(f2::pack(__uint_as_float(r[2]), __uint_as_float(r[3])), us2, a.y);
    out[2] = f2::fma(f2::pack(__uint_as_float(r[4]), __uint_as_float(r[5])), us2, b.x);
    out[3] = f2::fma(f2::pack(__uint_as_float(r[6]), __uint_as_float(r[7])), us2, b.y);
  }

  __device__ __forceinline__ void out_chunk(int j0, float (&out)[JC]) {
    uint32_t r[8];
    ptx::tmem_ld8(tm_lane + d_col() + j0, r);
    ptx::tmem_wait_ld();
    const float4* b4 = reinterpret_cast<const float4*>(img + L.off_bout + j0 * 4);
    const float4 a = b4[0], b = b4[1];
    const float bs[8] = {a.x, a.y, a.z, a.w, b.x, b.y, b.z, b.w};
    if (kF16) {
      const float us = unscale(L.nh + 1);
#pragma unroll
      for (int c = 0; c < 8; ++c) out[c] = fmaf(__uint_as_float(r[c]), us, bs[c]);
    } else {
#pragma unroll
      for (int c = 0; c < 8; ++c) out[c] = __uint_as_float(r[c]) + bs[c];
    }
  }
};

__host__ __device__ inline uint32_t tc_stage_bytes(const lrds_spec& s, int level) {
  return level > 0 ? (stage_layout(s, level).total + 15u) & ~15u : 0u;
}

template <int KIND, int PREC, int STAGE, class TR>
__global__ void __launch_bounds__(tc_max_warps(PREC) * 32, 1)
rollout_tc_kernel(const RolloutArgs a, const uint8_t* __restrict__ image, const uint32_t tmem_cols) {
  extern __shared__ __align__(128) uint8_t smem_raw[];
  const TcLayout TL = tc_layout(a.s.d, a.s.mlp.num_hidden, PREC);
  const int tid = threadIdx.x, warp = tid >> 5, nwarps = blockDim.x >> 5;
  uint64_t* bars = reinterpret_cast<uint64_t*>(smem_raw + TL.bytes);
  uint32_t* cnts = reinterpret_cast<uint32_t*>(smem_raw + TL.bytes + 64);
  uint8_t* stage = smem_raw + TL.bytes + TC_TAIL_BYTES;
  float* cols = reinterpret_cast<float*>(stage + tc_stage_bytes(a.s, STAGE));
  const uint32_t tmem = tc_cta_begin(smem_raw, TL, image, tmem_cols, warp, 5, nullptr, 0, cnts, 4, 0u, []() {});
  const int tile = warp >> 2;
  const int tile_warps = min(4, nwarps - 4 * tile);
  TcMlp<PREC> mlp;
  mlp.init(TL, smem_raw, tmem + (uint32_t)(tile * TL.tile_cols), warp, bars + 1 + tile, cnts + tile, (uint32_t)tile_warps,
           (warp & 3) == tile_warps - 1 ? 3u : 0u, a.s.mlp.d_pad);
  rollout_body<KIND, STAGE, TR>(a, cols, stage, mlp);
  tc_cta_end(warp, tmem, tmem_cols);
}

struct TcPlan {
  int warps, grid, staged;
  uint32_t tmem_cols;
  size_t smem;
};

inline int plan_warps(int need, int sms, int wmax) {
  const int waves = (need + sms * wmax - 1) / (sms * wmax);
  const int w = (need + sms * waves - 1) / (sms * waves);
  return w < 1 ? 1 : (w > wmax ? wmax : w);
}
inline uint32_t plan_tmem_cols(int cols) {
  uint32_t c = 32;
  while ((int)c < cols) c <<= 1;
  return c;
}

template <class K, class... A>
int launch_tc(K kernel, const char* what, const RolloutArgs& a, const TcPlan& p, int threads, cudaStream_t st, A... args) {
  cudaError_t e = cudaFuncSetAttribute(kernel, cudaFuncAttributeMaxDynamicSharedMemorySize, (int)p.smem);
  if (e == cudaSuccess) {
    kernel<<<p.grid, threads, p.smem, st>>>(a, static_cast<const uint8_t*>(a.s.mlp.tc_image), args...);
    e = cudaGetLastError();
  }
  if (e != cudaSuccess)
    return cuda_fail(e, "%s launch (grid %d x %d threads, %zu B smem, %u TMEM cols)", what, p.grid, threads, p.smem, p.tmem_cols);
  return LRDS_OK;
}

inline int plan_rollout_tc(const lrds_spec& s, int smem_cap, int sms, TcPlan* out, const char** why) {
  const TcLayout TL = tc_layout(s.d, s.mlp.num_hidden, s.precision);
  const ColLayout CL = col_layout(s);
  const size_t fixed = (size_t)TL.bytes + TC_TAIL_BYTES;
  const size_t per_warp = (size_t)CL.total * 32 * sizeof(float);
  if (TL.tile_cols > 512) { *why = "TMEM columns of one tile exceed 512"; return LRDS_ERR_RESOURCES; }
  if (fixed + per_warp > (size_t)smem_cap) { *why = "weight image + one warp of particle state exceed shared memory"; return LRDS_ERR_RESOURCES; }
  const int tmax = 512 / TL.tile_cols;
  const int need = (s.B + 31) / 32;
  auto pick = [&](size_t extra) {
    if (fixed + extra + per_warp > (size_t)smem_cap) return 0;
    int wmax = (int)(((size_t)smem_cap - fixed - extra) / per_warp);
    wmax = wmax < tc_max_warps(s.precision) ? wmax : tc_max_warps(s.precision);
    wmax = wmax < 4 * tmax ? wmax : 4 * tmax;
    return plan_warps(need, sms, wmax);
  };
  const int w_plain = pick(0);
  int level = 0, w = w_plain;
  size_t stage = 0;
  if (s.kind == LRDS_ROLLOUT_LINEAR) {
    for (int lv = 2; lv >= 1; --lv) {
      const size_t bytes = tc_stage_bytes(s, lv);
      const int wl = pick(bytes);
      if (wl >= w_plain) { level = lv; w = wl; stage = bytes; break; }
    }
  }
  const bool staged = level > 0;
  out->warps = w;
  out->grid = (need + w - 1) / w;
  out->staged = level;
  out->tmem_cols = plan_tmem_cols((w + 3) / 4 * TL.tile_cols);
  out->smem = fixed + (staged ? stage : 0) + per_warp * w;
  return LRDS_OK;
}

}
```

### sde_sampler_lrds_b200/csrc/lrds_tc_ptx.cuh

```cuda
#pragma once
#include <cuda_runtime.h>
#include <stdint.h>

namespace lrds {
namespace ptx {

__device__ __forceinline__ uint32_t smem_u32(const void* p) { return (uint32_t)__cvta_generic_to_shared(p); }

__device__ __forceinline__ void mbar_init(uint64_t* bar, uint32_t count) {
  asm volatile("mbarrier.init.shared::cta.b64 [%0], %1;" ::"r"(smem_u32(bar)), "r"(count) : "memory");
}
__device__ __forceinline__ void fence_mbar_init() { asm volatile("fence.mbarrier_init.release.cluster;" ::: "memory"); }
__device__ __forceinline__ void fence_proxy_async() { asm volatile("fence.proxy.async.shared::cta;" ::: "memory"); }
__device__ __forceinline__ void mbar_expect_tx(uint64_t* bar, uint32_t bytes) {
  asm volatile("mbarrier.arrive.expect_tx.shared::cta.b64 _, [%0], %1;" ::"r"(smem_u32(bar)), "r"(bytes) : "memory");
}
__device__ __forceinline__ void mbar_arrive(uint64_t* bar) {
  asm volatile("mbarrier.arrive.shared::cta.b64 _, [%0];" ::"r"(smem_u32(bar)) : "memory");
}
__device__ __forceinline__ bool mbar_try_wait(uint64_t* bar, uint32_t parity, uint32_t hint_ns = 2000u) {
  uint32_t ok;
  asm volatile(
      "{\n\t.reg .pred p;\n\t"
      "mbarrier.try_wait.parity.shared::cta.b64 p, [%1], %2, %3;\n\t"
      "selp.u32 %0, 1, 0, p;\n\t}"
      : "=r"(ok)
      : "r"(smem_u32(bar)), "r"(parity), "r"(hint_ns)
      : "memory");
  return ok != 0;
}
#ifndef LRDS_MBAR_WAIT_MODE
#define LRDS_MBAR_WAIT_MODE 0
#endif
__device__ __forceinline__ void mbar_wait(uint64_t* bar, uint32_t parity) {
#if LRDS_MBAR_WAIT_MODE == 0
  while (!mbar_try_wait(bar, parity)) {
  }
#elif LRDS_MBAR_WAIT_MODE == 1
  asm volatile(
      "{\n\t.reg .pred p;\n\t"
      "LRDS_WAIT_%=:\n\t"
      "mbarrier.try_wait.parity.shared::cta.b64 p, [%0], %1;\n\t"
      "@p bra LRDS_DONE_%=;\n\t"
      "bra LRDS_WAIT_%=;\n\t"
      "LRDS_DONE_%=:\n\t}" ::"r"(smem_u32(bar)),
      "r"(parity)
      : "memory");
#else
  uint32_t ok;
  for (;;) {
    asm volatile(
        "{\n\t.reg .pred p;\n\t"
        "mbarrier.test_wait.parity.shared::cta.b64 p, [%1], %2;\n\t"
        "selp.u32 %0, 1, 0, p;\n\t}"
        : "=r"(ok)
        : "r"(smem_u32(bar)), "r"(parity)
        : "memory");
    if (ok) break;
    asm volatile("nanosleep.u32 %0;" ::"r"((uint32_t)LRDS_MBAR_WAIT_MODE));
  }
#endif
}
__device__ __forceinline__ bool mbar_test(uint64_t* bar, uint32_t parity) {
  uint32_t ok;
  asm volatile(
      "{\n\t.reg .pred p;\n\t"
      "mbarrier.test_wait.parity.shared::cta.b64 p, [%1], %2;\n\t"
      "selp.u32 %0, 1, 0, p;\n\t}"
      : "=r"(ok)
      : "r"(smem_u32(bar)), "r"(parity)
      : "memory");
  return ok != 0;
}
__device__ __forceinline__ bool elect_one() {
  uint32_t pred;
  asm volatile(
      "{\n\t.reg .pred p;\n\t"
      "elect.sync _|p, 0xffffffff;\n\t"
      "selp.u32 %0, 1, 0, p;\n\t}"
      : "=r"(pred));
  return pred != 0;
}
__device__ __forceinline__ uint32_t atom_add_acq_rel(uint32_t* p, uint32_t v) {
  uint32_t old;
  asm volatile("atom.acq_rel.cta.shared::cta.add.u32 %0, [%1], %2;" : "=r"(old) : "r"(smem_u32(p)), "r"(v) : "memory");
  return old;
}
__device__ __forceinline__ void red_add_release(uint32_t* p, uint32_t v) {
  asm volatile("red.release.cta.shared::cta.add.u32 [%0], %1;" ::"r"(smem_u32(p)), "r"(v) : "memory");
}
__device__ __forceinline__ uint32_t ld_acquire(const uint32_t* p) {
  uint32_t v;
  asm volatile("ld.acquire.cta.shared::cta.u32 %0, [%1];" : "=r"(v) : "r"(smem_u32(p)) : "memory");
  return v;
}
__device__ __forceinline__ void nanosleep(uint32_t ns) { asm volatile("nanosleep.u32 %0;" ::"r"(ns)); }

__device__ __forceinline__ void bulk_g2s(void* dst_smem, const void* src_gmem, uint32_t bytes, uint64_t* bar) {
  asm volatile("cp.async.bulk.shared::cluster.global.mbarrier::complete_tx::bytes [%0], [%1], %2, [%3];" ::"r"(
                   smem_u32(dst_smem)),
               "l"(src_gmem), "r"(bytes), "r"(smem_u32(bar))
               : "memory");
}

__device__ __forceinline__ void bar_sync(int id, int nthreads) {
  asm volatile("bar.sync %0, %1;" ::"r"(id), "r"(nthreads) : "memory");
}

__device__ __forceinline__ void tmem_alloc(uint32_t* dst_smem, uint32_t ncols) {
  asm volatile("tcgen05.alloc.cta_group::1.sync.aligned.shared::cta.b32 [%0], %1;" ::"r"(smem_u32(dst_smem)), "r"(ncols)
               : "memory");
  asm volatile("tcgen05.relinquish_alloc_permit.cta_group::1.sync.aligned;" ::: "memory");
}
__device__ __forceinline__ void tmem_dealloc(uint32_t taddr, uint32_t ncols) {
  asm volatile("tcgen05.dealloc.cta_group::1.sync.aligned.b32 %0, %1;" ::"r"(taddr), "r"(ncols) : "memory");
}
__device__ __forceinline__ void tc_fence_before() { asm volatile("tcgen05.fence::before_thread_sync;" ::: "memory"); }
__device__ __forceinline__ void tc_fence_after() { asm volatile("tcgen05.fence::after_thread_sync;" ::: "memory"); }
__device__ __forceinline__ void tmem_wait_ld() { asm volatile("tcgen05.wait::ld.sync.aligned;" ::: "memory"); }
__device__ __forceinline__ void tmem_wait_st() { asm volatile("tcgen05.wait::st.sync.aligned;" ::: "memory"); }

__device__ __forceinline__ void tmem_ld8(uint32_t taddr, uint32_t (&r)[8]) {
  asm volatile("tcgen05.ld.sync.aligned.32x32b.x8.b32 {%0,%1,%2,%3,%4,%5,%6,%7}, [%8];"
               : "=r"(r[0]), "=r"(r[1]), "=r"(r[2]), "=r"(r[3]), "=r"(r[4]), "=r"(r[5]), "=r"(r[6]), "=r"(r[7])
               : "r"(taddr)
               : "memory");
}
__device__ __forceinline__ void tmem_ld16(uint32_t taddr, uint32_t (&r)[16]) {
  asm volatile(
      "tcgen05.ld.sync.aligned.32x32b.x16.b32 {%0,%1,%2,%3,%4,%5,%6,%7,%8,%9,%10,%11,%12,%13,%14,%15}, [%16];"
      : "=r"(r[0]), "=r"(r[1]), "=r"(r[2]), "=r"(r[3]), "=r"(r[4]), "=r"(r[5]), "=r"(r[6]), "=r"(r[7]), "=r"(r[8]),
        "=r"(r[9]), "=r"(r[10]), "=r"(r[11]), "=r"(r[12]), "=r"(r[13]), "=r"(r[14]), "=r"(r[15])
      : "r"(taddr)
      : "memory");
}
__device__ __forceinline__ void tmem_st8(uint32_t taddr, const uint32_t (&r)[8]) {
  asm volatile("tcgen05.st.sync.aligned.32x32b.x8.b32 [%0], {%1,%2,%3,%4,%5,%6,%7,%8};" ::"r"(taddr), "r"(r[0]),
               "r"(r[1]), "r"(r[2]), "r"(r[3]), "r"(r[4]), "r"(r[5]), "r"(r[6]), "r"(r[7])
               : "memory");
}
__device__ __forceinline__ void tmem_st16(uint32_t taddr, const uint32_t (&r)[16]) {
  asm volatile(
      "tcgen05.st.sync.aligned.32x32b.x16.b32 [%0], {%1,%2,%3,%4,%5,%6,%7,%8,%9,%10,%11,%12,%13,%14,%15,%16};" ::"r"(
          taddr),
      "r"(r[0]), "r"(r[1]), "r"(r[2]), "r"(r[3]), "r"(r[4]), "r"(r[5]), "r"(r[6]), "r"(r[7]), "r"(r[8]), "r"(r[9]),
      "r"(r[10]), "r"(r[11]), "r"(r[12]), "r"(r[13]), "r"(r[14]), "r"(r[15])
      : "memory");
}
__device__ __forceinline__ void tmem_ld32(uint32_t taddr, uint32_t (&r)[32]) {
  asm volatile("tcgen05.ld.sync.aligned.32x32b.x32.b32 {%0,%1,%2,%3,%4,%5,%6,%7,%8,%9,%10,%11,%12,%13,%14,%15,%16,%17,%18,%19,%20,%21,%22,%23,%24,%25,%26,%27,%28,%29,%30,%31}, [%32];"
               : "=r"(r[0]), "=r"(r[1]), "=r"(r[2]), "=r"(r[3]), "=r"(r[4]), "=r"(r[5]), "=r"(r[6]), "=r"(r[7]), "=r"(r[8]), "=r"(r[9]), "=r"(r[10]), "=r"(r[11]), "=r"(r[12]), "=r"(r[13]), "=r"(r[14]), "=r"(r[15]), "=r"(r[16]), "=r"(r[17]), "=r"(r[18]), "=r"(r[19]), "=r"(r[20]), "=r"(r[21]), "=r"(r[22]), "=r"(r[23]), "=r"(r[24]), "=r"(r[25]), "=r"(r[26]), "=r"(r[27]), "=r"(r[28]), "=r"(r[29]), "=r"(r[30]), "=r"(r[31])
               : "r"(taddr)
               : "memory");
}
__device__ __forceinline__ void tmem_st32(uint32_t taddr, const uint32_t (&r)[32]) {
  asm volatile("tcgen05.st.sync.aligned.32x32b.x32.b32 [%0], {%1,%2,%3,%4,%5,%6,%7,%8,%9,%10,%11,%12,%13,%14,%15,%16,%17,%18,%19,%20,%21,%22,%23,%24,%25,%26,%27,%28,%29,%30,%31,%32};" ::"r"(taddr),
               "r"(r[0]), "r"(r[1]), "r"(r[2]), "r"(r[3]), "r"(r[4]), "r"(r[5]), "r"(r[6]), "r"(r[7]), "r"(r[8]), "r"(r[9]), "r"(r[10]), "r"(r[11]), "r"(r[12]), "r"(r[13]), "r"(r[14]), "r"(r[15]), "r"(r[16]), "r"(r[17]), "r"(r[18]), "r"(r[19]), "r"(r[20]), "r"(r[21]), "r"(r[22]), "r"(r[23]), "r"(r[24]), "r"(r[25]), "r"(r[26]), "r"(r[27]), "r"(r[28]), "r"(r[29]), "r"(r[30]), "r"(r[31])
               : "memory");
}
__device__ __forceinline__ void tmem_st2(uint32_t taddr, uint32_t a, uint32_t b) {
  asm volatile("tcgen05.st.sync.aligned.32x32b.x2.b32 [%0], {%1,%2};" ::"r"(taddr), "r"(a), "r"(b) : "memory");
}
__device__ __forceinline__ void tmem_ld2(uint32_t taddr, uint32_t& a, uint32_t& b) {
  asm volatile("tcgen05.ld.sync.aligned.32x32b.x2.b32 {%0,%1}, [%2];" : "=r"(a), "=r"(b) : "r"(taddr) : "memory");
}

__device__ __forceinline__ uint64_t make_smem_desc(uint32_t saddr, uint32_t lbo_bytes, uint32_t sbo_bytes) {
  return (uint64_t)((saddr & 0x3FFFFu) >> 4) | ((uint64_t)(lbo_bytes >> 4) << 16) | ((uint64_t)(sbo_bytes >> 4) << 32) |
         (1ull << 46);
}
__host__ __device__ constexpr uint32_t make_idesc_tf32(int M, int N) {
  return (1u << 4) | (2u << 7) | (2u << 10) | ((uint32_t)(N >> 3) << 17) | ((uint32_t)(M >> 4) << 24);
}
__device__ __forceinline__ void mma_tf32_ts(uint32_t d_tmem, uint32_t a_tmem, uint64_t b_desc, uint32_t idesc,
                                            uint32_t accumulate) {
  asm volatile(
      "{\n\t.reg .pred p;\n\t"
      "setp.ne.b32 p, %4, 0;\n\t"
      "tcgen05.mma.cta_group::1.kind::tf32 [%0], [%1], %2, %3, p;\n\t}" ::"r"(d_tmem),
      "r"(a_tmem), "l"(b_desc), "r"(idesc), "r"(accumulate)
      : "memory");
}
__host__ __device__ constexpr uint32_t make_idesc_bf16(int M, int N) {
  return (1u << 4) | (1u << 7) | (1u << 10) | ((uint32_t)(N >> 3) << 17) | ((uint32_t)(M >> 4) << 24);
}
__device__ __forceinline__ void mma_bf16_ts(uint32_t d_tmem, uint32_t a_tmem, uint64_t b_desc, uint32_t idesc,
                                            uint32_t accumulate) {
  asm volatile(
      "{\n\t.reg .pred p;\n\t"
      "setp.ne.b32 p, %4, 0;\n\t"
      "tcgen05.mma.cta_group::1.kind::f16 [%0], [%1], %2, %3, p;\n\t}" ::"r"(d_tmem),
      "r"(a_tmem), "l"(b_desc), "r"(idesc), "r"(accumulate)
      : "memory");
}
__host__ __device__ constexpr uint32_t make_idesc_f16(int M, int N) {
  return (1u << 4) | ((uint32_t)(N >> 3) << 17) | ((uint32_t)(M >> 4) << 24);
}
__device__ __forceinline__ void mma_f16_ss(uint32_t d_tmem, uint64_t a_desc, uint64_t b_desc, uint32_t idesc,
                                           uint32_t accumulate) {
  asm volatile(
      "{\n\t.reg .pred p;\n\t"
      "setp.ne.b32 p, %4, 0;\n\t"
      "tcgen05.mma.cta_group::1.kind::f16 [%0], %1, %2, %3, p;\n\t}" ::"r"(d_tmem),
      "l"(a_desc), "l"(b_desc), "r"(idesc), "r"(accumulate)
      : "memory");
}
constexpr uint32_t IDESC_A_MN = 1u << 15, IDESC_B_MN = 1u << 16;
__device__ __forceinline__ void mma_commit(uint64_t* bar) {
  asm volatile("tcgen05.commit.cta_group::1.mbarrier::arrive::one.shared::cluster.b64 [%0];" ::"r"(smem_u32(bar))
               : "memory");
}

__device__ __forceinline__ float to_tf32(float v) {
  uint32_t r;
  asm("cvt.rna.tf32.f32 %0, %1;" : "=r"(r) : "f"(v));
  return __uint_as_float(r);
}

__device__ __forceinline__ uint32_t pack_bf16x2(float lo, float hi) {
  uint32_t r;
  asm("cvt.rn.bf16x2.f32 %0, %1, %2;" : "=r"(r) : "f"(hi), "f"(lo));
  return r;
}

__device__ __forceinline__ uint32_t pack_f16x2(float lo, float hi) {
  uint32_t r;
  asm("cvt.rn.satfinite.f16x2.f32 %0, %1, %2;" : "=r"(r) : "f"(hi), "f"(lo));
  return r;
}

}
}
```

Before: 3.281 billion.

## Split each particle across two threads using paired 16x32bx2 TMEM accesses

```diff
diff --git a/sde_sampler_lrds_b200/csrc/lrds_rollout_mix.cuh b/sde_sampler_lrds_b200/csrc/lrds_rollout_mix.cuh
--- a/sde_sampler_lrds_b200/csrc/lrds_rollout_mix.cuh
+++ b/sde_sampler_lrds_b200/csrc/lrds_rollout_mix.cuh
@@ -4,6 +4,7 @@
 namespace lrds {
 
 constexpr int MIX_MAX_WARPS = 16;
+constexpr int MIX_PAIR_SLOTS = 64;
 constexpr int MIX_TAIL_BYTES = 32;
 constexpr float MIX_LOGIT_KAPPA = 9.5367431640625e-07f;
 constexpr float MIX_LOGIT_KAPPA_C = 2.384185791015625e-07f;
@@ -48,7 +49,7 @@
 }
 __host__ __device__ inline bool mix_tc_applicable(const lrds_spec& s) { return mix_tc_config(s) >= 0; }
 
-__device__ __forceinline__ float gmm_logp_any(const GmmView& g, int d, int dp, const Col4& x) {
+__device__ __forceinline__ float gmm_logp_any(const GmmView& g, int d, int dp, const Col4& x, bool same = false) {
   if (g.M == 1) {
     const int nq = (d + 3) >> 2;
     float q = 0.f;
@@ -56,7 +57,7 @@
     return g.glogc.ld1(0) - 0.5f * q;
   }
   float r[MIX_MAX_M];
-  return gmm_pass1_pair(g, d, dp, x, r);
+  return gmm_pass1_pair(g, d, dp, x, r, same);
 }
 
 #ifdef LRDS_MIX_TIMING
@@ -130,6 +131,54 @@
     ptx::tmem_wait_ld();
   }
 
+  __device__ __forceinline__ void store_x_pair(const Col4& x, int h) {
+    for (int c0 = 0; c0 < this->L.Kin / 2; c0 += 8) {
+      const int j0 = 2 * c0 + 8 * h;
+      float4 va = make_float4(0.f, 0.f, 0.f, 0.f), vb = va;
+      if (j0 < this->dp) {
+        va = x.ld4(j0 >> 2);
+        vb = x.ld4((j0 >> 2) + 1);
+      }
+      const float v[8] = {va.x, va.y, va.z, va.w, vb.x, vb.y, vb.z, vb.w};
+      uint32_t ph[4], pl[4];
+#pragma unroll
+      for (int i = 0; i < 4; ++i) {
+        u64 hi, lo;
+        this->xmax = max3abs(this->xmax, v[2 * i], v[2 * i + 1]);
+        f2::split(f2::pack(v[2 * i], v[2 * i + 1]), hi, lo);
+        float h0, h1, l0, l1;
+        f2::unpack(hi, h0, h1);
+        f2::unpack(lo, l0, l1);
+        ph[i] = ptx::pack_f16x2(h0, h1);
+        pl[i] = ptx::pack_f16x2(l0, l1);
+      }
+      ptx::tmem_st4_pair<4>(this->tm_lane + this->a_col(0) + c0, ph);
+      ptx::tmem_st4_pair<4>(this->tm_lane + this->a_col(1) + c0, pl);
+    }
+  }
+  template <bool TGT, bool REF>
+  __device__ __forceinline__ void load_quarter(bool pair, int j0, int f, uint32_t (&m)[16], uint32_t (&u)[4]) {
+    const uint32_t col = pair ? 0u : 4u * (uint32_t)f;
+#pragma unroll
+    for (int i = 0; i < 4; ++i) {
+      uint32_t (&r)[4] = *reinterpret_cast<uint32_t(*)[4]>(m + 4 * i);
+      if ((i < 2 && TGT) || (i >= 2 && REF)) {
+        if (pair) ptx::tmem_ld4_pair<4>(this->tm_lane + kDCol + 8u * (uint32_t)i, r);
+        else ptx::tmem_ld4(this->tm_lane + kDCol + 8u * (uint32_t)i + col, r);
+      } else {
+        r[0] = r[1] = r[2] = r[3] = 0u;
+      }
+    }
+    if (pair) ptx::tmem_ld4_pair<4>(this->tm_lane + this->d_col() + (uint32_t)j0, u);
+    else ptx::tmem_ld4(this->tm_lane + this->d_col() + (uint32_t)j0 + col, u);
+  }
+  __device__ __forceinline__ void out_quad2(int j0, int f, const uint32_t (&u)[4], u64 (&out)[2]) const {
+    const ulonglong2 bb = *reinterpret_cast<const ulonglong2*>(this->img + this->L.off_bout + (j0 + 4 * f) * 4);
+    const u64 us2 = f2::pk(this->unscale(this->L.nh + 1));
+    out[0] = f2::fma(f2::pack(__uint_as_float(u[0]), __uint_as_float(u[1])), us2, bb.x);
+    out[1] = f2::fma(f2::pack(__uint_as_float(u[2]), __uint_as_float(u[3])), us2, bb.y);
+  }
+
   static __device__ __forceinline__ bool softmax_logits(const uint32_t* acc, const PPtr<true>& tail, float xnorm, uint32_t (&p)[16]) {
     float r[MIX_MAX_M];
     const float4 t2 = tail.ld4(MIX_MAX_M / 4);
@@ -161,7 +210,7 @@
   }
 
   template <bool BIAS_SH, class S0, class S1>
-  __device__ __forceinline__ void hidden_ws(const float* __restrict__ bias1, S0&& slot0, S1&& slot1) {
+  __device__ __forceinline__ void hidden_ws(const float* __restrict__ bias1, S0&& slot0, S1&& slot1, bool pair = false) {
     const TcLayout& L = this->L;
     this->issue(L.off_in, L.Kin, C);
     tm.mark(1);
@@ -176,7 +225,8 @@
       }
       this->wait();
       tm.mark(l == 0 ? 3 : l == 1 ? 6 : 8);
-      if (l == 0) this->template epilogue_f16<!BIAS_SH>(bias1, 0);
+      if (BIAS_SH && pair) this->template epilogue_f16<false, 16, true>(l == 0 ? bias1 : bh + (l - 1) * C, l);
+      else if (l == 0) this->template epilogue_f16<!BIAS_SH>(bias1, 0);
       else this->template epilogue_f16<false>(bh + (l - 1) * C, l);
       if (l < nh) this->issue(L.off_hid + (uint32_t)(l * C * C * L.es), C, C);
       else this->issue(L.off_out, C, L.Nout);
@@ -207,21 +257,24 @@
 
 template <int PREC, class CFG>
 __device__ __forceinline__ void rollout_body_mix(const RolloutArgs& a, float* smem, uint8_t* stage, uint32_t* step_cnt, const int nwarps,
-                                                 MixTc<PREC>& mlp) {
+                                                 const int ncol, const int nbody, const bool pair, MixTc<PREC>& mlp) {
   constexpr bool EUBO = CFG::kEubo, TMIX = CFG::kTgt == 1, TPHI = CFG::kTgt == 2, RMIX = CFG::kRef == 2, RGAUSS = CFG::kRef == 1, EM = CFG::kEm, DIS = CFG::kDis;
   const lrds_spec& s = a.s;
   const int NT = nwarps * 32;
-  const int tid = threadIdx.x;
-  const int b_raw = blockIdx.x * NT + tid;
-  const bool live = b_raw < s.B;
+  const int tid = threadIdx.x, lane = tid & 31;
+  const int h = pair ? lane >> 4 : 0;
+  const int slot = pair ? (tid >> 7) * 128 + ((tid >> 5) & 3) * 16 + (lane & 15) : tid;
+  const int b_raw = blockIdx.x * NT + slot;
+  const bool live = slot < NT && b_raw < s.B;
   const int b = live ? b_raw : s.B - 1;
   const int d = s.d, dp = s.mlp.d_pad, K = s.K;
   const ColLayout L = col_layout(s, true);
-  const Particle P = make_particle(smem, L, NT, tid);
-
-  for (int j = 0; j < dp; ++j) P.x(j) = (j < d) ? __ldg(a.x0 + (int64_t)b * d + j) : 0.f;
+  const Particle P = make_particle(smem, L, ncol, slot);
+  const int jstep = pair ? 2 : 1;
+
+  for (int j = h; j < dp; j += jstep) P.x(j) = (j < d) ? __ldg(a.x0 + (int64_t)b * d + j) : 0.f;
   if (!EUBO && a.traj_out != nullptr && live)
-    for (int j = 0; j < d; ++j) a.traj_out[(int64_t)b * d + j] = P.x(j);
+    for (int j = h; j < d; j += jstep) a.traj_out[(int64_t)b * d + j] = P.x(j);
 
   CtrlConst cc = ctrl_const(s);
   const GmmView tv0 = gmm_at(s.target.gmm, 0);
@@ -239,9 +292,9 @@
   mlp.lg_part = lg_part;
   auto target_logp = [&]() -> float {
     if (s.target.kind == LRDS_DISTR_GMM) {
-      if (s.target.gmm.M == 1) return gmm_logp_any(tv0, d, dp, P.x);
+      if (s.target.gmm.M == 1) return gmm_logp_any(tv0, d, dp, P.x, pair);
       float rt[MIX_MAX_M];
-      return gmm_pass1_pair(tv, d, dp, P.x, rt);
+      return gmm_pass1_pair(tv, d, dp, P.x, rt, pair);
     }
     if (s.target.kind == LRDS_DISTR_PHI4) return phi4_logp(s.target.phi4, d, P.x);
     return 0.f;
@@ -255,7 +308,7 @@
   __syncwarp();
   if constexpr (EUBO) {
     ptx::mbar_wait(sbar, 0);
-    const float lref = gmm_logp_any(gmm_at(s.ref_0, 0), d, dp, P.x);
+    const float lref = gmm_logp_any(gmm_at(s.ref_0, 0), d, dp, P.x, pair);
     rnd = lref - clipf(target_logp(), s.clip_target);
   }
 
@@ -277,18 +330,26 @@
 
     if constexpr (EUBO) {
       const u64 mean2 = f2::pk(rowp.ld1(LRDS_STEP_EU_A)), std2 = f2::pk(rowp.ld1(LRDS_STEP_EU_B));
+      auto quarter = [&](const int c, const int f) {
+        float z[4];
+        noise_quad(a, k, b, c * JC + 4 * f, z);
+        const ulonglong2 xv = P.x.ldu(2 * c + f);
+        P.x.stu(2 * c + f, ulonglong2{f2::fma(std2, f2::pack(z[0], z[1]), f2::mul(xv.x, mean2)),
+                                      f2::fma(std2, f2::pack(z[2], z[3]), f2::mul(xv.y, mean2))});
+      };
       for (int c = 0; c < nchunk; ++c) {
-        float z[JC];
-        noise_chunk(a, k, b, c * JC, z);
-        const ulonglong2 xa = P.x.ldu(2 * c), xb = P.x.ldu(2 * c + 1);
-        P.x.stu(2 * c, ulonglong2{f2::fma(std2, f2::pack(z[0], z[1]), f2::mul(xa.x, mean2)),
-                                  f2::fma(std2, f2::pack(z[2], z[3]), f2::mul(xa.y, mean2))});
-        P.x.stu(2 * c + 1, ulonglong2{f2::fma(std2, f2::pack(z[4], z[5]), f2::mul(xb.x, mean2)),
-                                      f2::fma(std2, f2::pack(z[6], z[7]), f2::mul(xb.y, mean2))});
-      }
-    }
-    mlp.store_x(P.x);
+        quarter(c, h);
+        if (!pair) quarter(c, 1);
+      }
+      if (pair) __syncwarp();
+    }
+    if (pair) mlp.store_x_pair(P.x, h);
+    else mlp.store_x(P.x);
     uint32_t rt_p[16], rr_p[16];
+    if constexpr (!(TMIX && RMIX)) {
+#pragma unroll
+      for (int i = 0; i < 16; ++i) rt_p[i] = rr_p[i] = 0u;
+    }
     bool need_t = TMIX, need_r = RMIX;
     bool ok_t = false, ok_r = false;
     if constexpr (TMIX || RMIX) {
@@ -308,16 +369,20 @@
         const float xnorm = sqrtf(f2::hsum1(n2));
         mlp.wait();
         uint32_t lg[32];
-        ptx::tmem_ld32(mlp.tm_lane + mlp.d_col(), lg);
+        if (pair) {
+          uint32_t l16[16];
+          ptx::tmem_ld16_pair<MIX_MAX_M>(mlp.tm_lane + mlp.d_col(), l16);
+#pragma unroll
+          for (int i = 0; i < 16; ++i) lg[i] = l16[i];
+        } else {
+          ptx::tmem_ld32(mlp.tm_lane + mlp.d_col(), lg);
+        }
         ptx::tmem_wait_ld();
-        if (lg_t) {
-          ok_t = mlp.softmax_logits(lg, tail_t, xnorm, rt_p);
-          need_t = __any_sync(0xffffffffu, !ok_t);
-        }
-        if (lg_r) {
-          ok_r = mlp.softmax_logits(lg + MIX_MAX_M, tail_r, xnorm, rr_p);
-          need_r = __any_sync(0xffffffffu, !ok_r);
-        }
+        if (pair ? (h ? lg_r : lg_t) : lg_t) ok_t = mlp.softmax_logits(lg, h ? tail_r : tail_t, xnorm, rt_p);
+        if (!pair && lg_r) ok_r = mlp.softmax_logits(lg + MIX_MAX_M, tail_r, xnorm, rr_p);
+        const uint32_t bad_t = __ballot_sync(0xffffffffu, !ok_t), bad_r = __ballot_sync(0xffffffffu, !ok_r);
+        if (lg_t) need_t = (pair ? bad_t & 0xffffu : bad_t) != 0u;
+        if (lg_r) need_r = (pair ? bad_t >> 16 : bad_r) != 0u;
       }
     }
     mlp.tm.count(14, need_t);
@@ -329,10 +394,11 @@
             if (need_t) {
               float r[MIX_MAX_M];
               uint32_t p[16];
-              gmm_pass1_pair(tv, d, dp, P.x, r);
+              gmm_pass1_pair(tv, d, dp, P.x, r, pair);
               mlp.pack_r(r, p);
-#pragma unroll
-              for (int i = 0; i < 16; ++i) rt_p[i] = ok_t ? rt_p[i] : p[i];
+              const bool keep = ok_t || h == 1;
+#pragma unroll
+              for (int i = 0; i < 16; ++i) rt_p[i] = keep ? rt_p[i] : p[i];
             }
           }
         },
@@ -341,15 +407,24 @@
             if (need_r) {
               float r[MIX_MAX_M];
               uint32_t p[16];
-              gmm_pass1_pair(rv, d, dp, P.x, r);
+              gmm_pass1_pair(rv, d, dp, P.x, r, pair);
               mlp.pack_r(r, p);
-#pragma unroll
-              for (int i = 0; i < 16; ++i) rr_p[i] = ok_r ? rr_p[i] : p[i];
+              const bool keep_t = !pair || ok_t || h == 0, keep_r = pair || ok_r;
+#pragma unroll
+              for (int i = 0; i < 16; ++i) {
+                rt_p[i] = keep_t ? rt_p[i] : p[i];
+                rr_p[i] = keep_r ? rr_p[i] : p[i];
+              }
             }
           }
-        });
-    if constexpr (TMIX) mlp.store_r(0, rt_p);
-    if constexpr (RMIX) mlp.store_r(1, rr_p);
+        },
+        pair);
+    if (pair) {
+      if constexpr (TMIX || RMIX) ptx::tmem_st16_pair<16>(mlp.tm_lane + MixTc<PREC>::kRCol, rt_p);
+    } else {
+      if constexpr (TMIX) mlp.store_r(0, rt_p);
+      if constexpr (RMIX) mlp.store_r(1, rr_p);
+    }
     mlp.arrive_issue([&]() { mlp.template chunk<TMIX, RMIX>(0, tgt_img, ref_img); });
     mlp.tm.mark(9);
     const float dt = EM ? rowp.ld1(LRDS_STEP_DT) : 0.f, sqdt = EM ? rowp.ld1(LRDS_STEP_SQRT_DT) : 0.f;
@@ -370,98 +445,131 @@
     float xm = 0.f;
     for (int c = 0; c < nchunk; ++c) {
       const int j0 = c * JC;
-      uint32_t m[32];
       mlp.wait();
       mlp.tm.mark(10);
-      mlp.load_chunk(m);
+      float xf[JC + 2];
+      if constexpr (TPHI) {
+        const ulonglong2 xa = P.x.ldu(2 * c), xb = P.x.ldu(2 * c + 1);
+        const u64 XC[4] = {xa.x, xa.y, xb.x, xb.y};
+        xf[0] = xm;
+#pragma unroll
+        for (int q = 0; q < 4; ++q) f2::unpack(XC[q], xf[1 + 2 * q], xf[2 + 2 * q]);
+        xf[JC + 1] = (j0 + JC < dp) ? P.x(j0 + JC) : 0.f;
+        xm = xf[JC];
+      }
+      u64 SV[2], SW[2], SZ[2], XN[2];
+      auto quarter = [&](const int f, const uint32_t (&m)[16], const uint32_t (&ur)[4]) {
+        u64 U[2];
+        mlp.out_quad2(j0, f, ur, U);
+        const ulonglong2 xv = P.x.ldu(2 * c + f);
+        const u64 X[2] = {xv.x, xv.y};
+        float z[4];
+        noise_quad(a, k, b, j0 + 4 * f, z);
+        float xs[6];
+        if constexpr (TPHI) {
+#pragma unroll
+          for (int i = 0; i < 6; ++i) xs[i] = f ? xf[4 + i] : xf[i];
+        }
+        u64 GM[2], GI[2];
+        if constexpr (RGAUSS || DIS) {
+          if (RGAUSS || lerp) {
+            const GmmView& gv = RGAUSS ? rg : pg;
+            const ulonglong2 g = gv.mu.ld2(2 * c + f), iv = gv.ivar.ld2(2 * c + f);
+            GM[0] = g.x; GM[1] = g.y;
+            GI[0] = iv.x; GI[1] = iv.y;
+          }
+        }
+#pragma unroll
+        for (int qi = 0; qi < 2; ++qi) {
+          const int q = 2 * f + qi;
+          const u64 ta = f2::pack(__uint_as_float(m[2 * qi]), __uint_as_float(m[2 * qi + 1]));
+          const u64 tb = f2::pack(__uint_as_float(m[4 + 2 * qi]), __uint_as_float(m[5 + 2 * qi]));
+          const u64 ra = f2::pack(__uint_as_float(m[8 + 2 * qi]), __uint_as_float(m[9 + 2 * qi]));
+          const u64 rb = f2::pack(__uint_as_float(m[12 + 2 * qi]), __uint_as_float(m[13 + 2 * qi]));
+          float t0 = 0.f, t1 = 0.f, u0, u1;
+          if constexpr (TMIX) f2::unpack(f2::fma(X[qi], ta, tb), t0, t1);
+          if constexpr (DIS) {
+            if (lerp) {
+              const u64 tt = f2::mul(f2::pack(t0, t1), ust2);
+              const u64 pr = f2::mul(f2::fma(X[qi], f2::pk(-1.0f), GM[qi]), GI[qi]);
+              const u64 df = f2::fma(pr, f2::pk(-1.0f), tt);
+              f2::unpack(f2::fma(df, wl2, wl < 0.5f ? pr : tt), t0, t1);
+            }
+          }
+          if constexpr (TPHI) {
+            const u64 nb = f2::pack(xs[2 * qi] + xs[2 * qi + 2], xs[2 * qi + 1] + xs[2 * qi + 3]);
+            const u64 t = f2::fma(X[qi], f2::fma(f2::mul(X[qi], X[qi]), p3, p1), f2::fma(pn, f2::fma(X[qi], m2, nb), p0));
+            f2::unpack(t, t0, t1);
+            if (j0 + JC > d) {
+              if (j0 + 2 * q >= d) t0 = 0.f;
+              if (j0 + 2 * q + 1 >= d) t1 = 0.f;
+            }
+          }
+          f2::unpack(U[qi], u0, u1);
+          const u64 uc = f2::pack(clipb(u0, cc.bound_model), clipb(u1, cc.bound_model));
+          u64 v = uc;
+          if constexpr (DIS) v = f2::fma(X[qi], cx2, v);
+          if constexpr (TMIX || TPHI) v = f2::fma(f2::pack(clipb(t0, bts), clipb(t1, bts)), gs2, v);
+          const u64 rraw = RMIX ? f2::fma(X[qi], ra, rb) : RGAUSS ? f2::mul(f2::fma(X[qi], f2::pk(-1.0f), GM[qi]), GI[qi]) : 0ull;
+          const u64 z2 = f2::pack(z[2 * qi], z[2 * qi + 1]);
+          const u64 w = EUBO ? f2::fma(v, f2::pk(0.5f), f2::mul(rraw, usr2)) : v;
+          SV[qi] = v;
+          SW[qi] = w;
+          SZ[qi] = z2;
+          if (!pair) {
+            su2 = f2::fma(v, w, su2);
+            sito = f2::fma(v, z2, sito);
+          }
+          if constexpr (EUBO) continue;
+          if constexpr (!RMIX && !RGAUSS) {
+            XN[qi] = f2::fma(C2, z2, f2::fma(A2, X[qi], f2::mul(B2, v)));
+          } else if constexpr (EM) {
+            XN[qi] = f2::fma(C2, z2, f2::fma(A2, X[qi], f2::fma(R2, rraw, f2::mul(B2, v))));
+          } else {
+            const u64 rv2 = f2::fma(rraw, usr2, v);
+            XN[qi] = f2::fma(C2, z2, f2::fma(A2, X[qi], f2::mul(B2, rv2)));
+          }
+        }
+        if constexpr (!EUBO) {
+          if (!pair) P.x.stu(2 * c + f, ulonglong2{XN[0], XN[1]});
+          if (a.traj_out != nullptr && live) {
+            float xn[4];
+            f2::unpack(XN[0], xn[0], xn[1]);
+            f2::unpack(XN[1], xn[2], xn[3]);
+            float* p = a.traj_out + ((int64_t)(k + 1) * s.B + b) * d + j0 + 4 * f;
+#pragma unroll
+            for (int i = 0; i < 4; ++i)
+              if (j0 + 4 * f + i < d) p[i] = xn[i];
+          }
+        }
+      };
+      uint32_t m0[16], m1[16], u0[4], u1[4];
+      mlp.template load_quarter<TMIX, RMIX>(pair, j0, h, m0, u0);
+      if (!pair) mlp.template load_quarter<TMIX, RMIX>(false, j0, 1, m1, u1);
+      ptx::tmem_wait_ld();
       if (c + 1 < nchunk) mlp.arrive_issue([&]() { mlp.template chunk<TMIX, RMIX>(c + 1, tgt_img, ref_img); });
       mlp.tm.mark(11);
-      const ulonglong2 xa = P.x.ldu(2 * c), xb = P.x.ldu(2 * c + 1);
-      const u64 X[4] = {xa.x, xa.y, xb.x, xb.y};
-      u64 U[4], XN[4];
-      float z[JC];
-      mlp.out_chunk2(j0, U);
-      noise_chunk(a, k, b, j0, z);
-      float xs[JC + 2];
-      if constexpr (TPHI) {
-        xs[0] = xm;
-#pragma unroll
-        for (int q = 0; q < 4; ++q) f2::unpack(X[q], xs[1 + 2 * q], xs[2 + 2 * q]);
-        xs[JC + 1] = (j0 + JC < dp) ? P.x(j0 + JC) : 0.f;
-        xm = xs[JC];
-      }
-      u64 GM[4], GI[4];
-      if constexpr (RGAUSS) {
-        const ulonglong2 g0 = rg.mu.ld2(2 * c), g1 = rg.mu.ld2(2 * c + 1), i0 = rg.ivar.ld2(2 * c), i1 = rg.ivar.ld2(2 * c + 1);
-        GM[0] = g0.x; GM[1] = g0.y; GM[2] = g1.x; GM[3] = g1.y;
-        GI[0] = i0.x; GI[1] = i0.y; GI[2] = i1.x; GI[3] = i1.y;
-      }
-      if constexpr (DIS) {
-        if (lerp) {
-          const ulonglong2 g0 = pg.mu.ld2(2 * c), g1 = pg.mu.ld2(2 * c + 1), i0 = pg.ivar.ld2(2 * c), i1 = pg.ivar.ld2(2 * c + 1);
-          GM[0] = g0.x; GM[1] = g0.y; GM[2] = g1.x; GM[3] = g1.y;
-          GI[0] = i0.x; GI[1] = i0.y; GI[2] = i1.x; GI[3] = i1.y;
+      quarter(h, m0, u0);
+      if (!pair) quarter(1, m1, u1);
+      if (pair) {
+        __syncwarp();
+        u64 PV[2], PW[2], PZ[2];
+#pragma unroll
+        for (int qi = 0; qi < 2; ++qi) {
+          PV[qi] = __shfl_xor_sync(0xffffffffu, SV[qi], 16);
+          PW[qi] = EUBO ? __shfl_xor_sync(0xffffffffu, SW[qi], 16) : PV[qi];
+          PZ[qi] = __shfl_xor_sync(0xffffffffu, SZ[qi], 16);
         }
-      }
-#pragma unroll
-      for (int q = 0; q < 4; ++q) {
-        const u64 ta = f2::pack(__uint_as_float(m[2 * q]), __uint_as_float(m[2 * q + 1]));
-        const u64 tb = f2::pack(__uint_as_float(m[8 + 2 * q]), __uint_as_float(m[9 + 2 * q]));
-        const u64 ra = f2::pack(__uint_as_float(m[16 + 2 * q]), __uint_as_float(m[17 + 2 * q]));
-        const u64 rb = f2::pack(__uint_as_float(m[24 + 2 * q]), __uint_as_float(m[25 + 2 * q]));
-        float t0 = 0.f, t1 = 0.f, u0, u1;
-        if constexpr (TMIX) f2::unpack(f2::fma(X[q], ta, tb), t0, t1);
-        if constexpr (DIS) {
-          if (lerp) {
-            const u64 tt = f2::mul(f2::pack(t0, t1), ust2);
-            const u64 pr = f2::mul(f2::fma(X[q], f2::pk(-1.0f), GM[q]), GI[q]);
-            const u64 df = f2::fma(pr, f2::pk(-1.0f), tt);
-            f2::unpack(f2::fma(df, wl2, wl < 0.5f ? pr : tt), t0, t1);
-          }
-        }
-        if constexpr (TPHI) {
-          const u64 nb = f2::pack(xs[2 * q] + xs[2 * q + 2], xs[2 * q + 1] + xs[2 * q + 3]);
-          const u64 t = f2::fma(X[q], f2::fma(f2::mul(X[q], X[q]), p3, p1), f2::fma(pn, f2::fma(X[q], m2, nb), p0));
-          f2::unpack(t, t0, t1);
-          if (j0 + JC > d) {
-            if (j0 + 2 * q >= d) t0 = 0.f;
-            if (j0 + 2 * q + 1 >= d) t1 = 0.f;
-          }
-        }
-        f2::unpack(U[q], u0, u1);
-        const u64 uc = f2::pack(clipb(u0, cc.bound_model), clipb(u1, cc.bound_model));
-        u64 v = uc;
-        if constexpr (DIS) v = f2::fma(X[q], cx2, v);
-        if constexpr (TMIX || TPHI) v = f2::fma(f2::pack(clipb(t0, bts), clipb(t1, bts)), gs2, v);
-        const u64 rraw = RMIX ? f2::fma(X[q], ra, rb) : RGAUSS ? f2::mul(f2::fma(X[q], f2::pk(-1.0f), GM[q]), GI[q]) : 0ull;
-        const u64 z2 = f2::pack(z[2 * q], z[2 * q + 1]);
-        if constexpr (EUBO) {
-          su2 = f2::fma(v, f2::fma(v, f2::pk(0.5f), f2::mul(rraw, usr2)), su2);
-          sito = f2::fma(v, z2, sito);
-          continue;
-        }
-        su2 = f2::fma(v, v, su2);
-        sito = f2::fma(v, z2, sito);
-        if constexpr (!RMIX && !RGAUSS) {
-          XN[q] = f2::fma(C2, z2, f2::fma(A2, X[q], f2::mul(B2, v)));
-        } else if constexpr (EM) {
-          XN[q] = f2::fma(C2, z2, f2::fma(A2, X[q], f2::fma(R2, rraw, f2::mul(B2, v))));
-        } else {
-          const u64 rv2 = f2::fma(rraw, usr2, v);
-          XN[q] = f2::fma(C2, z2, f2::fma(A2, X[q], f2::mul(B2, rv2)));
-        }
-      }
-      if constexpr (EUBO) {
-        mlp.tm.mark(12);
-        continue;
-      }
-      P.x.stu(2 * c, ulonglong2{XN[0], XN[1]});
-      P.x.stu(2 * c + 1, ulonglong2{XN[2], XN[3]});
-      if (a.traj_out != nullptr && live) {
-        float xn[JC];
-#pragma unroll
-        for (int q = 0; q < 4; ++q) f2::unpack(XN[q], xn[2 * q], xn[2 * q + 1]);
-        store_traj(a, k + 1, b, j0, xn);
+#pragma unroll
+        for (int g = 0; g < 2; ++g)
+#pragma unroll
+          for (int qi = 0; qi < 2; ++qi) {
+            const bool own = g == h;
+            const u64 v = own ? SV[qi] : PV[qi];
+            su2 = f2::fma(v, own ? SW[qi] : PW[qi], su2);
+            sito = f2::fma(v, own ? SZ[qi] : PZ[qi], sito);
+          }
+        if constexpr (!EUBO) P.x.stu(2 * c + h, ulonglong2{XN[0], XN[1]});
       }
       mlp.tm.mark(12);
     }
@@ -475,27 +583,30 @@
     __syncwarp();
     if ((tid & 31) == 0) {
       const uint32_t old = ptx::atom_add_acq_rel(step_cnt + (k & 1), 1u);
-      if (old == (uint32_t)((k >> 1) * nwarps + nwarps - 1) && k + 2 < K) mix_load_step<RMIX>(s, SL, stage, k + 2);
+      if (old == (uint32_t)((k >> 1) * nbody + nbody - 1) && k + 2 < K) mix_load_step<RMIX>(s, SL, stage, k + 2);
     }
     mlp.tm.mark(13);
   }
   __syncwarp();
   if constexpr (!EUBO) {
-    const float lref = s.init_cost ? a.rnd_out[b] : gmm_logp_any(gmm_at(s.ref_0, 0), d, dp, P.x);
+    const float lref = s.init_cost ? a.rnd_out[b] : gmm_logp_any(gmm_at(s.ref_0, 0), d, dp, P.x, pair);
     rnd += lref - clipf(target_logp(), s.clip_target);
   }
+  if (pair) __syncwarp();
 
   float xsum = 0.f;
   if (live) {
-    a.rnd_out[b] = rnd;
+    if (h == 0) a.rnd_out[b] = rnd;
     if (a.x_out != nullptr)
       for (int j = 0; j < d; ++j) {
         const float v = P.x(j);
         xsum += v;
-        a.x_out[(int64_t)b * d + j] = v;
-      }
-  }
-  report_status(s, live, mlp.saturated(), !isfinite(rnd + xsum));
+        if (!pair || (j & 1) == h) a.x_out[(int64_t)b * d + j] = v;
+      }
+  }
+  bool sat = mlp.saturated();
+  if (pair) sat = __shfl_xor_sync(0xffffffffu, (int)sat, 16) != 0 || sat;
+  report_status(s, live && h == 0, sat, !isfinite(rnd + xsum));
 }
 
 template <int PREC, class CFG>
@@ -535,6 +646,12 @@
   }
 }
 
+__host__ __device__ constexpr bool mix_paired(int w) { return w % 4 == 1 || w % 4 == 2; }
+__host__ __device__ constexpr int mix_cta_warps(int w) {
+  return mix_paired(w) ? w / 4 * 4 + 4 : w + ((w % 4 != 0 && w < MIX_MAX_WARPS) ? 1 : 0);
+}
+__host__ __device__ constexpr int mix_col_warps(int w) { return mix_paired(w) ? w / 4 * 4 + MIX_PAIR_SLOTS / 32 : w; }
+
 template <int PREC, class CFG>
 __global__ void __launch_bounds__(MIX_MAX_WARPS * 32, 1)
 rollout_mix_kernel(const RolloutArgs a, const uint8_t* __restrict__ image, const uint32_t tmem_cols, const int nwarps) {
@@ -544,33 +661,37 @@
   const TcLayout TL = tc_layout(s.d, s.mlp.num_hidden, PREC);
   const int tid = threadIdx.x;
   const int warp = __shfl_sync(0xffffffffu, tid >> 5, 0);
-  const bool has_aux = (int)(blockDim.x >> 5) > nwarps;
+  const int cta_warps = (int)(blockDim.x >> 5);
+  const bool paired = mix_paired(nwarps);
+  const bool has_aux = !paired && cta_warps > nwarps;
   uint64_t* bars = reinterpret_cast<uint64_t*>(smem_raw + TL.bytes);
   uint32_t* cnts = reinterpret_cast<uint32_t*>(smem_raw + TL.bytes + TC_TAIL_BYTES);
   uint8_t* stage = smem_raw + TL.bytes + TC_TAIL_BYTES + MIX_TAIL_BYTES;
   const StageLayout SL = stage_layout(s, 2, true);
   float* cols = reinterpret_cast<float*>(stage + ((SL.total + 15u) & ~15u));
+  const int ncol = 32 * mix_col_warps(nwarps);
   auto steps01 = [&]() {
     for (int k = 0; k < 2 && k < s.K; ++k) mix_load_step<RMIX>(s, SL, stage, k);
   };
   const uint32_t tmem = __shfl_sync(
       0xffffffffu, tc_cta_begin(smem_raw, TL, image, tmem_cols, warp, 5, reinterpret_cast<uint64_t*>(stage), 2, cnts, 6, 0u, steps01), 0);
-  const bool aux = warp == nwarps;
+  const bool aux = has_aux && warp == nwarps;
   const int tile = aux ? (nwarps - 1) >> 2 : warp >> 2;
-  const int tile_warps = min(4, nwarps - 4 * tile);
+  const int tile_warps = min(4, (paired ? cta_warps : nwarps) - 4 * tile);
+  const bool pair = paired && tile == nwarps / 4;
   uint32_t issue_mask = ((warp & 3) == tile_warps - 1 ? 1u : 0u) | ((warp & 3) == max(tile_warps - 2, 0) ? 2u : 0u);
   if (has_aux && tile_warps < 4) issue_mask = 0u;
   MixTc<PREC> mlp;
   mlp.init(TL, smem_raw, tmem + (uint32_t)(tile * TL.tile_cols), warp, bars + 1 + tile, cnts + tile, (uint32_t)tile_warps, issue_mask,
            s.mlp.d_pad);
 #ifdef LRDS_MIX_TIMING
-  unsigned long long* tmw = reinterpret_cast<unsigned long long*>(cols + (size_t)col_layout(s, true).total * 32 * nwarps) + warp * 16;
+  unsigned long long* tmw = reinterpret_cast<unsigned long long*>(cols + (size_t)col_layout(s, true).total * ncol) + warp * 16;
   if ((tid & 31) < 16) tmw[tid & 31] = 0;
   __syncwarp();
   mlp.tm.w = tmw;
 #endif
   if (aux) mix_aux_issuer<PREC, CFG>(a, stage, mlp);
-  else rollout_body_mix<PREC, CFG>(a, cols, stage, cnts + 4, nwarps, mlp);
+  else rollout_body_mix<PREC, CFG>(a, cols, stage, cnts + 4, nwarps, ncol, paired ? cta_warps : nwarps, pair, mlp);
 #ifdef LRDS_MIX_TIMING
   __syncwarp();
   if ((blockIdx.x == 0 || blockIdx.x == gridDim.x / 2) && (tid & 31) < 16)
@@ -589,24 +710,24 @@
   fixed += 16 * 16 * 8;
 #endif
   const size_t per_warp = (size_t)CL.total * 32 * sizeof(float);
-  if (fixed + per_warp > (size_t)smem_cap) return false;
+  if (fixed + per_warp * mix_col_warps(1) > (size_t)smem_cap) return false;
   int wmax = (int)(((size_t)smem_cap - fixed) / per_warp);
   wmax = wmax < MIX_MAX_WARPS ? wmax : MIX_MAX_WARPS;
   wmax = wmax < 4 * (512 / TL.tile_cols) ? wmax : 4 * (512 / TL.tile_cols);
+  while (fixed + per_warp * mix_col_warps(wmax) > (size_t)smem_cap) --wmax;
   const int need = (s.B + 31) / 32;
   const int w = plan_warps(need, sms, wmax);
   out->warps = w;
   out->grid = (need + w - 1) / w;
   out->staged = 2;
   out->tmem_cols = plan_tmem_cols((w + 3) / 4 * TL.tile_cols);
-  out->smem = fixed + per_warp * w;
+  out->smem = fixed + per_warp * mix_col_warps(w);
   return true;
 }
 
 template <class CFG>
 int launch_mix_cfg(const RolloutArgs& a, const TcPlan& p, cudaStream_t st) {
-  const int aux = (p.warps % 4 != 0 && p.warps < MIX_MAX_WARPS) ? 1 : 0;
-  return launch_tc(rollout_mix_kernel<LRDS_PRECISION_F16X3, CFG>, "mixture tensor-core rollout", a, p, (p.warps + aux) * 32, st,
+  return launch_tc(rollout_mix_kernel<LRDS_PRECISION_F16X3, CFG>, "mixture tensor-core rollout", a, p, mix_cta_warps(p.warps) * 32, st,
                    p.tmem_cols, p.warps);
 }
 
diff --git a/sde_sampler_lrds_b200/csrc/lrds_rollout_simt.cuh b/sde_sampler_lrds_b200/csrc/lrds_rollout_simt.cuh
--- a/sde_sampler_lrds_b200/csrc/lrds_rollout_simt.cuh
+++ b/sde_sampler_lrds_b200/csrc/lrds_rollout_simt.cuh
@@ -255,14 +255,15 @@
 constexpr int MIX_MAX_M = 16;
 
 template <bool SH>
-__device__ __forceinline__ float gmm_pass1_pair(const GmmViewT<SH>& g, int d, int dp, const Col4& x, float (&r)[MIX_MAX_M]) {
+__device__ __forceinline__ float gmm_pass1_pair(const GmmViewT<SH>& g, int d, int dp, const Col4& x, float (&r)[MIX_MAX_M],
+                                                bool same = false) {
   const int lane = threadIdx.x & 31, h = lane >> 4;
   const int nq = (d + 3) >> 2;
   const int rowq = dp >> 2;
   const int M4 = (g.M + 3) >> 2;
   const int nb = (M4 + 1) >> 1;
   const int b0 = h * nb;
-  const Col4 xo{x.p + ((lane ^ 16) - lane) * 4, x.stride};
+  const Col4 xo{same ? x.p : x.p + ((lane ^ 16) - lane) * 4, x.stride};
   const int blk0 = min(b0, M4 - 1), blk1 = min(b0 + 1, M4 - 1);
   PPtr<SH> p0 = g.sn + blk0 * rowq * 32, p1 = g.sn + blk1 * rowq * 32;
   u64 qa[8] = {0, 0, 0, 0, 0, 0, 0, 0}, qb[8] = {0, 0, 0, 0, 0, 0, 0, 0};
@@ -400,6 +401,21 @@
 #pragma unroll
       for (int c = 0; c < JC; ++c)
         if (j0 + c >= a.s.d) z[c] = 0.f;
+    }
+  }
+}
+
+__device__ __forceinline__ void noise_quad(const RolloutArgs& a, int step, int b, int j4, float (&z)[4]) {
+  if (a.noise != nullptr) {
+    const float* p = a.noise + ((int64_t)step * a.s.B + b) * a.s.d + j4;
+#pragma unroll
+    for (int c = 0; c < 4; ++c) z[c] = (j4 + c < a.s.d) ? __ldg(p + c) : 0.f;
+  } else {
+    normals4(a.seed, (uint32_t)(a.particle_offset + (uint64_t)b), (uint32_t)step, (uint32_t)(j4 >> 2), 0u, z);
+    if (j4 + 4 > a.s.d) {
+#pragma unroll
+      for (int c = 0; c < 4; ++c)
+        if (j4 + c >= a.s.d) z[c] = 0.f;
     }
   }
 }
diff --git a/sde_sampler_lrds_b200/csrc/lrds_rollout_tc.cuh b/sde_sampler_lrds_b200/csrc/lrds_rollout_tc.cuh
--- a/sde_sampler_lrds_b200/csrc/lrds_rollout_tc.cuh
+++ b/sde_sampler_lrds_b200/csrc/lrds_rollout_tc.cuh
@@ -302,17 +302,20 @@
     }
   }
 
-  template <bool GLOBAL_BIAS, int W = 32>
+  template <bool GLOBAL_BIAS, int W = 32, bool PAIR = false>
   __device__ __forceinline__ void epilogue_f16(const float* __restrict__ bias, int layer, int c_begin = 0, int c_end = C) {
     static_assert(W == 32 || W == 16, "tcgen05.ld / st widths");
+    static_assert(!PAIR || W == 16, "the paired epilogue takes 16 columns per thread");
     const u64 us2 = f2::pk(unscale(layer));
 #pragma unroll 1
-    for (int c0 = c_begin; c0 < c_end; c0 += W) {
+    for (int c0 = c_begin; c0 < c_end; c0 += PAIR ? 2 * W : W) {
       uint32_t r[W];
-      if constexpr (W == 32) ptx::tmem_ld32(tm_lane + d_col() + c0, r);
+      if constexpr (PAIR) ptx::tmem_ld16_pair<16>(tm_lane + d_col() + c0, r);
+      else if constexpr (W == 32) ptx::tmem_ld32(tm_lane + d_col() + c0, r);
       else ptx::tmem_ld16(tm_lane + d_col() + c0, r);
       ptx::tmem_wait_ld();
-      const float4* b4 = reinterpret_cast<const float4*>(bias + c0);
+      const int cb = PAIR ? c0 + W * (int)((threadIdx.x >> 4) & 1) : c0;
+      const float4* b4 = reinterpret_cast<const float4*>(bias + cb);
       uint32_t ph[W / 2], pl[W / 2];
 #pragma unroll
       for (int i = 0; i < W / 4; ++i) {
@@ -336,7 +339,10 @@
           pl[2 * i + e] = ptx::pack_f16x2(l0, l1);
         }
       }
-      if constexpr (W == 32) {
+      if constexpr (PAIR) {
+        ptx::tmem_st8_pair<W / 2>(tm_lane + a_col(0) + c0 / 2, ph);
+        ptx::tmem_st8_pair<W / 2>(tm_lane + a_col(1) + c0 / 2, pl);
+      } else if constexpr (W == 32) {
         ptx::tmem_st16(tm_lane + a_col(0) + c0 / 2, ph);
         ptx::tmem_st16(tm_lane + a_col(1) + c0 / 2, pl);
       } else {
diff --git a/sde_sampler_lrds_b200/csrc/lrds_tc_ptx.cuh b/sde_sampler_lrds_b200/csrc/lrds_tc_ptx.cuh
--- a/sde_sampler_lrds_b200/csrc/lrds_tc_ptx.cuh
+++ b/sde_sampler_lrds_b200/csrc/lrds_tc_ptx.cuh
@@ -126,6 +126,12 @@
                : "r"(taddr)
                : "memory");
 }
+__device__ __forceinline__ void tmem_ld4(uint32_t taddr, uint32_t (&r)[4]) {
+  asm volatile("tcgen05.ld.sync.aligned.32x32b.x4.b32 {%0,%1,%2,%3}, [%4];"
+               : "=r"(r[0]), "=r"(r[1]), "=r"(r[2]), "=r"(r[3])
+               : "r"(taddr)
+               : "memory");
+}
 __device__ __forceinline__ void tmem_ld16(uint32_t taddr, uint32_t (&r)[16]) {
   asm volatile(
       "tcgen05.ld.sync.aligned.32x32b.x16.b32 {%0,%1,%2,%3,%4,%5,%6,%7,%8,%9,%10,%11,%12,%13,%14,%15}, [%16];"
@@ -158,6 +164,42 @@
                "r"(r[0]), "r"(r[1]), "r"(r[2]), "r"(r[3]), "r"(r[4]), "r"(r[5]), "r"(r[6]), "r"(r[7]), "r"(r[8]), "r"(r[9]), "r"(r[10]), "r"(r[11]), "r"(r[12]), "r"(r[13]), "r"(r[14]), "r"(r[15]), "r"(r[16]), "r"(r[17]), "r"(r[18]), "r"(r[19]), "r"(r[20]), "r"(r[21]), "r"(r[22]), "r"(r[23]), "r"(r[24]), "r"(r[25]), "r"(r[26]), "r"(r[27]), "r"(r[28]), "r"(r[29]), "r"(r[30]), "r"(r[31])
                : "memory");
 }
+template <int OFF>
+__device__ __forceinline__ void tmem_ld4_pair(uint32_t taddr, uint32_t (&r)[4]) {
+  asm volatile("tcgen05.ld.sync.aligned.16x32bx2.x4.b32 {%0,%1,%2,%3}, [%4], %5;"
+               : "=r"(r[0]), "=r"(r[1]), "=r"(r[2]), "=r"(r[3])
+               : "r"(taddr), "n"(OFF)
+               : "memory");
+}
+template <int OFF>
+__device__ __forceinline__ void tmem_ld16_pair(uint32_t taddr, uint32_t (&r)[16]) {
+  asm volatile(
+      "tcgen05.ld.sync.aligned.16x32bx2.x16.b32 {%0,%1,%2,%3,%4,%5,%6,%7,%8,%9,%10,%11,%12,%13,%14,%15}, [%16], %17;"
+      : "=r"(r[0]), "=r"(r[1]), "=r"(r[2]), "=r"(r[3]), "=r"(r[4]), "=r"(r[5]), "=r"(r[6]), "=r"(r[7]), "=r"(r[8]),
+        "=r"(r[9]), "=r"(r[10]), "=r"(r[11]), "=r"(r[12]), "=r"(r[13]), "=r"(r[14]), "=r"(r[15])
+      : "r"(taddr), "n"(OFF)
+      : "memory");
+}
+template <int OFF>
+__device__ __forceinline__ void tmem_st4_pair(uint32_t taddr, const uint32_t (&r)[4]) {
+  asm volatile("tcgen05.st.sync.aligned.16x32bx2.x4.b32 [%0], %1, {%2,%3,%4,%5};" ::"r"(taddr), "n"(OFF), "r"(r[0]), "r"(r[1]),
+               "r"(r[2]), "r"(r[3])
+               : "memory");
+}
+template <int OFF>
+__device__ __forceinline__ void tmem_st8_pair(uint32_t taddr, const uint32_t (&r)[8]) {
+  asm volatile("tcgen05.st.sync.aligned.16x32bx2.x8.b32 [%0], %1, {%2,%3,%4,%5,%6,%7,%8,%9};" ::"r"(taddr), "n"(OFF), "r"(r[0]),
+               "r"(r[1]), "r"(r[2]), "r"(r[3]), "r"(r[4]), "r"(r[5]), "r"(r[6]), "r"(r[7])
+               : "memory");
+}
+template <int OFF>
+__device__ __forceinline__ void tmem_st16_pair(uint32_t taddr, const uint32_t (&r)[16]) {
+  asm volatile(
+      "tcgen05.st.sync.aligned.16x32bx2.x16.b32 [%0], %1, {%2,%3,%4,%5,%6,%7,%8,%9,%10,%11,%12,%13,%14,%15,%16,%17};" ::"r"(taddr),
+      "n"(OFF), "r"(r[0]), "r"(r[1]), "r"(r[2]), "r"(r[3]), "r"(r[4]), "r"(r[5]), "r"(r[6]), "r"(r[7]), "r"(r[8]), "r"(r[9]),
+      "r"(r[10]), "r"(r[11]), "r"(r[12]), "r"(r[13]), "r"(r[14]), "r"(r[15])
+      : "memory");
+}
 __device__ __forceinline__ void tmem_st2(uint32_t taddr, uint32_t a, uint32_t b) {
   asm volatile("tcgen05.st.sync.aligned.32x32b.x2.b32 [%0], {%1,%2};" ::"r"(taddr), "r"(a), "r"(b) : "memory");
 }
```

Result: slower. 2.343 billion, median of 6 (-28.6%).
